# apache/paimon

Measured on NVIDIA H100. Metric: merged rows/sec at 16 runs x 40M rows, higher is better.
Workload: dtype int64

## Files before the change

paimon_b200/csrc/api.cu:

```cuda
#include <algorithm>
#include <atomic>
#include <cstdlib>
#include <cstring>
#include <map>
#include <memory>
#include <mutex>
#include <queue>

#include "pg_internal.h"

namespace pg {

static thread_local std::string g_last_error;
void set_error(const std::string &msg) { g_last_error = msg; }
pg_status fail(pg_status code, const std::string &msg) {
    g_last_error = msg;
    return code;
}

static int g_device = -1;

struct Arena {
    unsigned char *base = nullptr;
    size_t cap = 0;
// ... 334 lines not shown
    for (int c = 0; c < nc; c++) any |= read[c] && is_varlen(schema->field(c).type);
    if (!any) return PG_OK;
    for (int r = 0; r < (int)run_rows.size(); r++) {
        OutColumn *o = &out[(size_t)r * nc];
        const int64_t *bytes = &payload[(size_t)r * nc];
        auto carve = [&](void *base) {
            Carver cv(base);
            for (int c = 0; c < nc; c++)
                if (read[c] && is_varlen(schema->field(c).type)) o[c].data = cv.take<uint8_t>((size_t)bytes[c] + kReadPast);
            return cv.bytes();
        };
        const size_t total = carve(nullptr);
        Run &run = *scratch.runs[r];
        run.bufs.emplace_back(total);
        unsigned char *pl = run.bufs.back().get();
        if (!pl) return oom(who, "the var-len payload of a run", total);
        carve(pl);
        for (int c = 0; c < nc; c++) {
            if (!read[c] || !is_varlen(schema->field(c).type)) continue;
            run.varlen_bytes[c] = bytes[c];
            decoded_bytes += bytes[c];
        }
    }
    return PG_OK;
}

void RunBuilder::finish(uint64_t *out_runs, int64_t bytes_h2d, pg_section_info *info) {
    const int n_runs = (int)run_rows.size();
    for (int r = 0; r < n_runs; r++) {
        Run &run = *scratch.runs[r];
        for (int c = 0; c < nc; c++) {
            const OutColumn &o = out[(size_t)r * nc + c];
            if (read[c]) run.cols[c] = DevColumn{o.data ? o.data : run.bufs[0].get(), o.offsets, (const uint8_t *)o.validity};
        }
        run.bytes_h2d = r == 0 ? bytes_h2d : 0;
        out_runs[r] = g_runs.put(std::move(scratch.runs[r]));
    }
    if (info) {
        memset(info, 0, sizeof(*info));
        for (int64_t n : run_rows) info->n_rows += n;
        info->n_runs = n_runs;
        info->decoded_bytes = decoded_bytes;
    }
}

SectionFrame::SectionFrame(std::shared_ptr<const Schema> s, int n_runs, const char *who)
    : stream(copy_stream()), scratch(stream), b(std::move(s), n_runs, scratch, who) {}

pg_status SectionFrame::start(const uint8_t *read_cols, const char *const *names) {
    PG_CUDA(cudaEventCreate(&tm.e0));
    PG_CUDA(cudaEventCreate(&tm.e1));
    PG_CUDA(cudaEventRecord(tm.e0, stream));
    return b.read_columns(read_cols, names);
}

pg_status SectionFrame::place(const pg_file_desc *files, int n_files) {
    d_file.assign(n_files, nullptr);
    for (int f = 0; f < n_files; f++) {
        file_bytes += files[f].size;
        if (files[f].mem == PG_MEM_DEVICE) { d_file[f] = files[f].bytes; continue; }
        { pg_status st = file_image(scratch, files[f].bytes, files[f].size, b.who, &d_file[f]); if (st) return st; }
        h2d += files[f].size;
    }
    return PG_OK;
}

pg_status SectionFrame::finish(const int32_t *d_err, uint64_t *out_runs, pg_section_info *info) {
    PG_CUDA(cudaEventRecord(tm.e1, stream));
    int32_t herr = 0;
    SmallReads rb(stream);
    { pg_status rs = rb.add(&herr, d_err, 4); if (!rs) rs = rb.finish(); if (rs) return rs; }
    PG_CUDA(cudaGetLastError());
    { pg_status st = kernel_error(herr, b.who); if (st) return st; }
    b.finish(out_runs, h2d, info);
    if (info) {
        info->file_bytes = file_bytes;
        info->page_bytes = page_bytes;
        info->n_files = (int32_t)d_file.size();
        info->launches = launches;
        info->ms_decode = tm.ms();
    }
    return PG_OK;
}

static void free_outputs(Merge *m, bool release_memory = false) {
    m->out_cols.clear();
    m->has_batch = false;
    if (release_memory) {
        if (m->stream) cudaStreamSynchronize(m->stream);
        m->outbuf.release();
    }
}


static bool agg_supports_retract(int agg) {
    return agg == PG_AGG_SUM || agg == PG_AGG_PRODUCT || agg == PG_AGG_LAST_VALUE ||
           agg == PG_AGG_LAST_NON_NULL_VALUE || agg == PG_AGG_PRIMARY_KEY;
}

static pg_status build_descriptors(Merge *m) {
    const Schema *s = m->spec->schema.get();
    const Spec *sp = m->spec.get();
    if (s->n_key < 1 || s->n_key > PG_MAX_KEY_FIELDS)
        return fail(PG_ERR_UNSUPPORTED, "more than 4 primary-key fields are not implemented on the device");
    m->key = KeyDesc{};
    m->key.n_fields = s->n_key;
    int key_bytes = 0;
    bool all_fixed = true;
    for (int f = 0; f < s->n_key; f++) {
        int t = s->key_fields[f].type;
        if (t == PG_FLOAT || t == PG_DOUBLE)
            return fail(PG_ERR_UNSUPPORTED, "FLOAT / DOUBLE primary keys are not implemented on the device "
                                            "(the reference's comparator treats NaN as equal to everything)");
        m->key.type[f] = t;
        m->key.width[f] = type_width(t);
        if (is_varlen(t)) all_fixed = false;
        key_bytes += type_width(t);
    }
    m->key.exact = all_fixed && key_bytes <= 8;
    m->seq = SeqFields{};
    if (sp->seq_fields.size() > 4)
        return fail(PG_ERR_UNSUPPORTED, "more than 4 'sequence.field' columns are not implemented on the device");
    for (size_t i = 0; i < sp->seq_fields.size(); i++) {
        int vf = sp->seq_fields[i];
        if (vf < 0 || vf >= s->n_val) return fail(PG_ERR_INVALID, "sequence.field index out of range");
        int t = s->val_fields[vf].type;
        if (is_varlen(t))
            return fail(PG_ERR_UNSUPPORTED, "var-len 'sequence.field' columns are not implemented on the device");
        m->seq.col[i] = s->n_key + 2 + vf;
        m->seq.type[i] = t;
        m->seq.width[i] = type_width(t);
    }
    m->seq.n = (int32_t)sp->seq_fields.size();
    m->seq.ascending = sp->seq_ascending ? 1 : 0;
    m->flags = MergeFlags{sp->engine, sp->ignore_delete, sp->remove_record_on_delete, sp->drop_delete};

    const int nc = s->n_cols();
    m->cols.assign(nc, ColDesc{});
    m->varlen_cols.clear();
    m->emit.assign(nc, 1);
    for (int c = s->n_key + 2; c < nc; c++)
        if (!sp->read_fields.empty() && !sp->read_fields[c - s->n_key - 2]) m->emit[c] = 0;
    std::vector<uint8_t> needed = m->emit;
    for (int32_t vf : sp->seq_fields) if (vf >= 0 && vf < s->n_val) needed[s->n_key + 2 + vf] = 1;
    for (int32_t vf : sp->group_seq_fields) if (vf >= 0 && vf < s->n_val) needed[s->n_key + 2 + vf] = 1;
    for (int r = 0; r < m->k; r++)
        for (int c = 0; c < nc; c++)
            if (needed[c] && m->runs[r]->n_rows > 0 && !m->runs[r]->cols[c].data && !m->runs[r]->cols[c].offsets)
                return fail(PG_ERR_INVALID, "run " + std::to_string(r) + " has no buffers for column " + std::to_string(c) +
                                            ", which the merge reads (read-type projection dropped a field the merge "
                                            "function compares or emits)");
    for (int c = 0; c < nc; c++) {
        pg_field f = s->field(c);
        ColDesc &cd = m->cols[c];
        cd.type = f.type;
        cd.width = type_width(f.type);
        cd.nullable = f.nullable;
        cd.agg = PG_AGG_NONE;
        cd.retract = RT_OK;
        cd.varlen_index = -1;
        cd.decimal = 0;
        if (is_varlen(f.type) && m->emit[c]) {
            cd.varlen_index = (int)m->varlen_cols.size();
            m->varlen_cols.push_back(c);
        }
        if (c < s->n_key) { cd.mode = CM_KEY; cd.nullable = 0; }
        else if (c == s->n_key) { cd.mode = CM_SEQ; cd.nullable = 0; }
        else if (c == s->n_key + 1) { cd.mode = CM_KIND; cd.nullable = 0; }
        else {
            int vi = c - s->n_key - 2;
            int agg = sp->agg.empty() ? PG_AGG_NONE : sp->agg[vi];
            bool ign = !sp->ignore_retract.empty() && sp->ignore_retract[vi];
            const int32_t dec = sp->decimal.empty() ? 0 : sp->decimal[vi];
            const int32_t fold_dec = agg == PG_AGG_SUM || agg == PG_AGG_PRODUCT ? dec : 0;
            if (sp->engine == PG_ENGINE_AGGREGATE) {
                if (agg == PG_AGG_NONE) agg = PG_AGG_LAST_NON_NULL_VALUE;
                bool numeric = f.type == PG_INT8 || f.type == PG_INT16 || f.type == PG_INT32 ||
                               f.type == PG_INT64 || f.type == PG_FLOAT || f.type == PG_DOUBLE;
                if ((agg == PG_AGG_SUM || agg == PG_AGG_PRODUCT) && !numeric)
                    return fail(PG_ERR_INVALID, "sum/product need a numeric column");
                if ((agg == PG_AGG_BOOL_AND || agg == PG_AGG_BOOL_OR) && f.type != PG_BOOL)
                    return fail(PG_ERR_INVALID, "bool_and/bool_or need a BOOLEAN column");
                if ((agg == PG_AGG_MAX || agg == PG_AGG_MIN) && f.type == PG_BOOL)
                    return fail(PG_ERR_INVALID, "Incomparable type: BOOLEAN");
                if (agg < PG_AGG_SUM || agg > PG_AGG_PRIMARY_KEY)
                    return fail(PG_ERR_UNSUPPORTED, "aggregate function not implemented on the device");
                cd.mode = CM_FOLD;
                cd.agg = agg;
                cd.decimal = fold_dec;
                cd.nullable = 1;
                cd.retract = ign ? RT_IGNORE : (agg_supports_retract(agg) ? RT_OK : RT_ERROR);
            } else {
                const bool in_group = sp->n_groups() > 0 && sp->field_group[vi] >= 0;
                if (sp->engine == PG_ENGINE_PARTIAL_UPDATE && !in_group && agg != PG_AGG_NONE &&
                    agg != PG_AGG_LAST_NON_NULL_VALUE && agg != PG_AGG_PRIMARY_KEY)
                    return fail(PG_ERR_INVALID, "Must use sequence group for aggregation functions");
                cd.mode = CM_SELECT;
                if (sp->n_groups() > 0 && sp->field_group[vi] >= 0) {
                    const int g = sp->field_group[vi];
                    bool is_seq = false;
                    for (int j = sp->group_seq_start[g]; j < sp->group_seq_start[g + 1]; j++)
                        if (sp->group_seq_fields[j] == vi) is_seq = true;
                    cd.mode = is_seq ? CM_GSEQ : CM_GVAL;
                    cd.agg = g;
                    cd.nullable = 1;
                    if (!is_seq && agg != PG_AGG_NONE) {
                        cd.mode = CM_GAGG;
                        cd.agg = agg;
                        cd.decimal = fold_dec;
                        cd.group = g;
                        cd.retract = ign ? RT_IGNORE : (agg_supports_retract(agg) ? RT_OK : RT_ERROR);
                        m->has_group_aggs = true;
                    }
                }
            }
        }
    }

    const int k = m->k, nk = s->n_key, nv = (int)m->varlen_cols.size();
    MergeDesc h;
    const size_t total = h.carve(nullptr, k, nk, nc, nv);
    std::vector<unsigned char> host(total, 0);
    h.carve(host.data(), k, nk, nc, nv);
    m->varlen_bound.assign(nv, 0);
    for (int r = 0; r < k; r++) {
        const Run *run = m->runs[r].get();
        for (int f = 0; f < nk; f++) {
            h.key_ptrs[r * nk + f] = run->cols[f].data;
            h.key_offs[r * nk + f] = run->cols[f].offsets;
        }
        h.seq_ptrs[r] = (const int64_t *)run->cols[nk].data;
        h.kind_ptrs[r] = (const int8_t *)run->cols[nk + 1].data;
        for (int c = 0; c < nc; c++) {
            h.data[(size_t)c * k + r] = run->cols[c].data;
            h.offsets[(size_t)c * k + r] = run->cols[c].offsets;
            h.validity[(size_t)c * k + r] = (const uint32_t *)run->cols[c].validity;
            if (m->cols[c].varlen_index >= 0) m->varlen_bound[m->cols[c].varlen_index] += run->varlen_bytes[c];
        }
        h.run_rows[r] = run->n_rows;
    }
    memcpy(h.cols, m->cols.data(), sizeof(ColDesc) * nc);
    {
        int n = 0;
        for (int c = 0; c < nc; c++) if (m->emit[c] && m->cols[c].width == 0) h.col_order[n++] = c;
        for (int c = 0; c < nc; c++) if (m->emit[c] && m->cols[c].width != 0) h.col_order[n++] = c;
        m->n_passes = n;
        for (int v = 0; v < nv; v++) h.varlen_cols[v] = m->varlen_cols[v];
    }
    if (sp->n_groups() > 0) {
        SeqGroups *sg = h.groups;
        sg->n = sp->n_groups();
        for (int g = 0; g <= sg->n; g++) sg->start[g] = sp->group_seq_start[g];
        for (int j = 0; j < sp->group_seq_start[sg->n]; j++) {
            const int vf = sp->group_seq_fields[j];
            sg->col[j] = s->n_key + 2 + vf;
            sg->type[j] = s->val_fields[vf].type;
            sg->width[j] = type_width(s->val_fields[vf].type);
        }
        for (int g = 0; g < sg->n; g++) sg->partial_delete[g] = sp->group_partial_delete[g];
    }
    if (!m->d_desc || total > m->desc_cap) {
        if (m->d_desc) cudaFree(m->d_desc);
        m->d_desc = nullptr;
        PG_CUDA(cudaMalloc(&m->d_desc, total));
        m->desc_cap = total;
    }
    { pg_status ts = small_h2d(m->d_desc, host.data(), total, m->stream, m->ring); if (ts) return ts; }
    PG_CUDA(cudaStreamSynchronize(m->stream));
    m->desc.carve(m->d_desc, k, nk, nc, nv);
    if (sp->n_groups() == 0) m->desc.groups = nullptr;
    if (!m->h_totals) PG_CUDA(cudaMallocHost((void **)&m->h_totals, sizeof(int64_t) * (nv + 1) + 16));
    m->h_err = (int32_t *)(m->h_totals + nv + 1);
    return PG_OK;
}

pg_status kernel_error(int code, const char *who) {
    static const struct { int code; pg_status st; const char *msg; } kErrors[] = {
        {KERR_PU_DELETE, PG_ERR_MERGE_FUNCTION,
         "By default, Partial update can not accept delete records, you can choose one of the "
         "following solutions:\n1. Configure 'ignore-delete' to ignore delete records.\n"
         "2. Configure 'partial-update.remove-record-on-delete' to remove the whole row when "
         "receiving delete records.\n3. Configure 'sequence-group's to retract partial columns. "
         "Also configure 'partial-update.remove-record-on-sequence-group' to remove the whole "
         "row when receiving deleted records of `specified sequence group`."},
        {KERR_FIRST_ROW_RETRACT, PG_ERR_MERGE_FUNCTION,
         "By default, First row merge engine can not accept DELETE/UPDATE_BEFORE records.\n"
         "You can config 'ignore-delete' to ignore the DELETE/UPDATE_BEFORE records."},
        {KERR_AGG_RETRACT, PG_ERR_MERGE_FUNCTION,
         "Aggregate function does not support retraction, If you allow this function to ignore "
         "retraction messages, you can configure 'fields.${field_name}.ignore-retract'='true'."},
        {KERR_DIV_ZERO, PG_ERR_MERGE_FUNCTION, "ArithmeticException: / by zero"},
        {KERR_DEC_DIV_ZERO, PG_ERR_MERGE_FUNCTION, "ArithmeticException: Division by zero"},
        {KERR_DEC_DIV_UNDEFINED, PG_ERR_MERGE_FUNCTION, "ArithmeticException: Division undefined"},
        {KERR_DEC_NON_TERMINATING, PG_ERR_MERGE_FUNCTION,
         "ArithmeticException: Non-terminating decimal expansion; no exact representable decimal result."},
        {KERR_TILE_OVERFLOW, PG_ERR_INTERNAL,
         "a merge tile overflowed (does a run contain duplicate keys? SortMergeReader.java:37 requires unique keys per reader)"},
        {KERR_OFFSET_OVERFLOW, PG_ERR_INTERNAL, "a var-len column exceeds 2 GiB of payload"},
        {KERR_BAD_PAGE, PG_ERR_FORMAT, "a page or stream does not decode (malformed file or unsupported encoding)"},
        {KERR_PQ_HEADER, PG_ERR_FORMAT, "malformed or truncated page header"},
        {KERR_PQ_NO_DICT, PG_ERR_FORMAT, "dictionary-encoded page without dictionary"},
        {KERR_PQ_ROWS, PG_ERR_FORMAT, "page row counts do not add up"},
        {KERR_PQ_DICT_ID, PG_ERR_FORMAT, "dictionary id outside the dictionary"},
        {KERR_PQ_ENCODING, PG_ERR_UNSUPPORTED,
         "a page uses a value encoding the device decoder does not implement (PLAIN, dictionary, DELTA_BINARY_PACKED "
         "integers and RLE booleans are decoded)"},
        {KERR_PQ_LEVELS, PG_ERR_UNSUPPORTED, "repetition levels / BIT_PACKED definition levels are not decoded on device"},
    };
    if (code == KERR_NONE) return PG_OK;
    for (const auto &e : kErrors)
        if (e.code == code) return fail(e.st, e.st == PG_ERR_MERGE_FUNCTION ? std::string(e.msg) : std::string(who) + ": " + e.msg);
    return fail(PG_ERR_INTERNAL, std::string(who) + ": unknown kernel error " + std::to_string(code));
}


static pg_status execute(Merge *m) {
    pg_status st = ensure_device();
    if (st) return st;
    cudaStream_t sm = m->stream;
    PG_HOST_MARKS("merge execute");
    free_outputs(m);
    for (size_t r = m->runs.size(); r < m->bound.size(); r++)
        if (!m->runs.emplace_back(m->bound[r].lock())) {
            m->runs.clear();
            return fail(PG_ERR_INVALID, "a run of this merge has been freed since it was merged: rebind first");
        }
    const Schema *s = m->spec->schema.get();
    const int k = m->k, nc = s->n_cols(), nv = (int)m->varlen_cols.size();
    m->stats = pg_stats{};
    m->stats.rows_in = m->n_in;
    int launches = 0;

    const int S = kSampleStride;
    const int q = kPlanTile / S - 2 * k;
    if (q < 1) return fail(PG_ERR_UNSUPPORTED, "too many runs for one merge call");
    std::vector<LevelView> views;
    std::vector<int64_t> level_total;
    {
        int64_t stride = 1;
        while (true) {
            LevelView lv{};
            lv.stride = stride;
            int64_t tot = 0;
            for (int r = 0; r < k; r++) {
                lv.row0[r] = m->row0[r];
                lv.count[r] = (m->runs[r]->n_rows - m->row0[r]) / stride;
                tot += lv.count[r];
            }
            views.push_back(lv);
            level_total.push_back(tot);
            if (tot <= kPlanTile) break;
            stride *= S;
        }
    }
    const int top = (int)views.size() - 1;
    std::vector<int> n_tiles(top + 1);
    n_tiles[top] = 1;
    for (int l = top - 1; l >= 0; l--) n_tiles[l] = (int)((level_total[l + 1] + q - 1) / q);
    m->stats.n_levels = top;
    m->stats.n_tiles = n_tiles[0];

    PG_CUDA(cudaMemsetAsync(m->desc.err, 0, sizeof(int32_t), sm));
    PG_CUDA(cudaEventRecord(m->ev[0], sm));

    MergeLaunch ml{k, m->key, KeySrc{m->desc.key_ptrs, m->desc.key_offs}, sm, m->desc.err, nullptr};
    const int T = n_tiles[0];
    int64_t N = m->n_in;
    for (int r = 0; r < k; r++) N += m->row0[r];
    int *d_skip = nullptr;
    std::vector<int64_t *> bounds(top + 1);
    std::vector<uint64_t *> sk(top + 1), sref(top + 1);
    uint16_t *plan = nullptr;
    uint32_t *gplan = nullptr, *gagg = nullptr;
    int32_t *tile_rows = nullptr;
    int64_t *tmp_seq = nullptr, *row_base = nullptr;
    int8_t *tmp_kind = nullptr;
    uint64_t *vl_state = nullptr;
    const size_t vl_words = (size_t)T * std::max(nv, 1);
    auto carve_work = [&](void *base) {
        Carver cv(base);
        if (!m->key.exact) d_skip = cv.take<int>(1);
        for (int l = top; l >= 0; l--) {
            bounds[l] = cv.take<int64_t>((size_t)(n_tiles[l] + 1) * k);
            if (l > 0) {
                sk[l] = cv.take<uint64_t>((size_t)std::max<int64_t>(level_total[l], 1));
                sref[l] = cv.take<uint64_t>((size_t)std::max<int64_t>(level_total[l], 1));
            }
        }
        plan = cv.take<uint16_t>((size_t)N + 8);
        if (m->desc.groups) gplan = cv.take<uint32_t>((size_t)N + 4);
        if (m->has_group_aggs) gagg = cv.take<uint32_t>((size_t)N + 4);
        tile_rows = cv.take<int32_t>(T);
        tmp_seq = cv.take<int64_t>((size_t)N + 2);
        tmp_kind = cv.take<int8_t>((size_t)N + 16);
        row_base = cv.take<int64_t>(T);
        vl_state = cv.take<uint64_t>(vl_words);
        return cv.bytes();
    };
    PG_CUDA(m->work.reserve(carve_work(nullptr)));
    carve_work(m->work.base);

    if (!m->key.exact) {
        launch_key_lcp(ml, views[0], d_skip);
        ml.skip = d_skip;
        launches++;
    }
    for (int l = top; l >= 0; l--) {
        launch_partition(ml, views[l], l < top ? sk[l + 1] : nullptr, l < top ? sref[l + 1] : nullptr, q, n_tiles[l],
                         bounds[l]);
        launches++;
        if (l > 0) {
            launch_merge_keys(ml, views[l], bounds[l], n_tiles[l], sk[l], sref[l]);
            launches++;
        }
    }
    PG_CUDA(cudaEventRecord(m->ev[1], sm));

    PG_CUDA(cudaMemsetAsync(vl_state, 0, sizeof(uint64_t) * vl_words, sm));
    PG_CUDA(cudaMemsetAsync(m->desc.tile_counter, 0, sizeof(int32_t), sm));

    PlanArgs pa{};
    pa.bounds = bounds[0];
    pa.n_tiles = T;
    pa.seq_ptrs = m->desc.seq_ptrs;
    pa.kind_ptrs = m->desc.kind_ptrs;
    pa.flags = m->flags;
    pa.seq = m->seq;
    pa.ptrs = m->desc.ptrs();
    pa.plan = plan;
    pa.tile_rows = tile_rows;
    pa.tmp_seq = tmp_seq;
    pa.tmp_kind = tmp_kind;
    pa.groups = m->desc.groups;
    pa.gplan = gplan;
    pa.gagg = gagg;
    launch_plan(ml, pa);
    launch_scan(sm, tile_rows, T, row_base, m->desc.totals);
    launches += 2;
    PG_CUDA(cudaEventRecord(m->ev[2], sm));
    PG_HOST_MARK("enqueue");
    {
        SmallReads rb(sm);
        pg_status rs = rb.add(m->h_totals, m->desc.totals, sizeof(int64_t));
        if (!rs) rs = rb.add(m->h_err, m->desc.err, sizeof(int32_t));
        if (!rs) rs = rb.finish();
        if (rs) return rs;
    }
    if (*m->h_err != KERR_NONE) return kernel_error(*m->h_err, "merge");
    PG_HOST_MARK("size_readback");

    const int64_t n_out = m->h_totals[0];
    m->n_out = n_out;
    m->out_cols.assign(nc, pg_out_column{});
    size_t vspan = 0;
    int64_t bytes_out = 0;
    auto carve_out = [&](void *base) {
        Carver cv(base);
        bytes_out = 0;
        for (int c = 0; c < nc; c++)
            if (m->cols[c].nullable && m->emit[c]) {
                m->out_cols[c].validity = cv.take<uint8_t>((size_t)((n_out + 31) / 32) * 4 + kReadPast);
                bytes_out += (n_out + 7) / 8;
            }
        vspan = cv.bytes();
        for (int c = 0; c < nc; c++) {
            const ColDesc &cd = m->cols[c];
            pg_out_column &oc = m->out_cols[c];
            if (!m->emit[c]) continue;
            if (cd.width > 0) {
                oc.data_bytes = n_out * cd.width;
                oc.data = cv.take<uint8_t>((size_t)oc.data_bytes + kReadPast);
                bytes_out += oc.data_bytes;
            } else {
                oc.data_bytes = m->varlen_bound[cd.varlen_index];
                oc.data = cv.take<uint8_t>((size_t)oc.data_bytes + kReadPast);
                oc.offsets = cv.take<int32_t>((size_t)n_out + 1 + kReadPast / 4);
                bytes_out += 4 * (n_out + 1);
            }
        }
        return cv.bytes();
    };
    PG_CUDA(m->outbuf.reserve(carve_out(nullptr)));
    carve_out(m->outbuf.base);
    if (vspan) PG_CUDA(cudaMemsetAsync(m->outbuf.base, 0, vspan, sm));
    m->stats.bytes_out = bytes_out;
    { pg_status ts = small_h2d(m->desc.out_cols, m->out_cols.data(), sizeof(pg_out_column) * nc, sm, m->ring); if (ts) return ts; }

    EmitArgs ea{};
    ea.bounds = bounds[0];
    ea.n_tiles = (T + 1) / 2;
    ea.n_plan_tiles = T;
    ea.tile_rows = tile_rows;
    ea.k = k;
    ea.plan = plan;
    ea.row_base = row_base;
    ea.tmp_seq = tmp_seq;
    ea.tmp_kind = tmp_kind;
    ea.gplan = gplan;
    ea.gagg = gagg;
    ea.cols = m->desc.cols;
    ea.col_order = m->desc.col_order;
    ea.n_passes = m->n_passes;
    ea.varlen_cols = m->desc.varlen_cols;
    ea.ptrs = m->desc.ptrs();
    ea.run_rows = m->desc.run_rows;
    ea.n_cols = nc;
    ea.n_varlen = nv;
    ea.out_cols = m->desc.out_cols;
    ea.totals = m->desc.totals;
    ea.vl_state = vl_state;
    ea.tile_counter = m->desc.tile_counter;
    ea.err = m->desc.err;
    ea.stream = sm;
    PG_CUDA(cudaEventRecord(m->ev[4], sm));
    launch_emit(ea);
    launches++;
    PG_CUDA(cudaEventRecord(m->ev[3], sm));
    PG_HOST_MARK("alloc_emit");
    {
        SmallReads rb(sm);
        pg_status rs = rb.add(m->h_err, m->desc.err, sizeof(int32_t));
        if (!rs) rs = rb.add(m->h_totals, m->desc.totals, sizeof(int64_t) * (nv + 1));
        if (!rs) rs = rb.finish();
        if (rs) return rs;
    }
    PG_CUDA(cudaGetLastError());
    PG_HOST_MARK("emit_readback");
    m->has_batch = true;
    if (*m->h_err != KERR_NONE) {
        free_outputs(m);
        return kernel_error(*m->h_err, "merge");
    }
    for (int c = 0; c < nc; c++)
        if (m->cols[c].width == 0 && m->emit[c]) {
            m->out_cols[c].data_bytes = m->h_totals[1 + m->cols[c].varlen_index];
            m->stats.bytes_out += m->out_cols[c].data_bytes;
        }
    m->stats.rows_out = n_out;
    m->stats.launches = launches;
    cudaEventElapsedTime(&m->stats.ms_partition, m->ev[0], m->ev[1]);
    cudaEventElapsedTime(&m->stats.ms_plan, m->ev[1], m->ev[2]);
    cudaEventElapsedTime(&m->stats.ms_alloc, m->ev[2], m->ev[4]);
    cudaEventElapsedTime(&m->stats.ms_emit, m->ev[4], m->ev[3]);
    cudaEventElapsedTime(&m->stats.ms_total, m->ev[0], m->ev[3]);
    m->runs.clear();
    return PG_OK;
}

}


using namespace pg;

extern "C" {

const char *pg_last_error(void) { return g_last_error.c_str(); }
int32_t pg_abi_version(void) { return PG_ABI_VERSION; }

pg_status pg_init(int32_t device_ordinal) {
    int n = 0;
    cudaError_t e = cudaGetDeviceCount(&n);
    if (e != cudaSuccess || n == 0)
        return fail(PG_ERR_CUDA, std::string("no CUDA device: libpaimon_gpu has no CPU fallback (") +
                                     cudaGetErrorString(e) + ")");
    if (device_ordinal < 0 || device_ordinal >= n) return fail(PG_ERR_INVALID, "bad device ordinal");
    if (g_device >= 0 && g_device != device_ordinal)
        return fail(PG_ERR_INVALID, "pg_init: this process is already bound to device " + std::to_string(g_device) +
                                    " (one process per GPU: handles, streams and cached buffers belong to it)");
    PG_CUDA(cudaSetDevice(device_ordinal));
    g_device = device_ordinal;
    cudaMemPool_t pool;
    PG_CUDA(cudaDeviceGetDefaultMemPool(&pool, device_ordinal));
    uint64_t thr = UINT64_MAX;
    PG_CUDA(cudaMemPoolSetAttribute(pool, cudaMemPoolAttrReleaseThreshold, &thr));
    return PG_OK;
}

pg_status pg_shutdown(void) {
    if (g_device >= 0) {
        cudaSetDevice(g_device);
        cudaDeviceSynchronize();
        buf_trim(0);
        cudaMemPool_t pool;
        if (cudaDeviceGetDefaultMemPool(&pool, g_device) == cudaSuccess) cudaMemPoolTrimTo(pool, 0);
    }
    return PG_OK;
}

pg_status pg_schema_create(const pg_schema_desc *desc, uint64_t *out_schema) {
    if (!desc || !out_schema) return fail(PG_ERR_INVALID, "null argument");
    if (desc->n_key < 1 || desc->n_val < 0 || desc->n_key + 2 + desc->n_val > kMaxCols)
        return fail(PG_ERR_INVALID, "bad field counts");
    auto s = std::make_unique<Schema>();
    s->n_key = desc->n_key;
    s->n_val = desc->n_val;
    for (int i = 0; i < desc->n_key; i++) {
        if (!type_ok(desc->key_fields[i].type)) return fail(PG_ERR_INVALID, "bad key field type");
        s->key_fields.push_back(pg_field{desc->key_fields[i].type, 0});
    }
    for (int i = 0; i < desc->n_val; i++) {
        if (!type_ok(desc->val_fields[i].type)) return fail(PG_ERR_INVALID, "bad value field type");
        s->val_fields.push_back(desc->val_fields[i]);
    }
    *out_schema = g_schemas.put(std::move(s));
    return PG_OK;
}
// ... 493 lines not shown
```

paimon_b200/csrc/parquet_decode.cu:

```cuda
#include <algorithm>
#include <cstring>
#include <memory>
#include <stdexcept>

#include "device_utils.cuh"
#include "parquet_meta.h"
#include "inflate_device.cuh"
#include "lz4_device.cuh"
#include "snappy_device.cuh"
#include "scan_kernels.cuh"
#include "zstd_device.cuh"

namespace pg {

enum : int { ENC_PLAIN = 0, ENC_DICT = 1, ENC_DELTA_BP = 2, ENC_RLE_BOOL = 3 };

struct PqChunk {
    const uint8_t *base;
    int64_t avail;
    int64_t num_values;
    int64_t row0;
    int32_t col, run, file, codec;
    int32_t max_def, phys, phys_width;
    int32_t cast;
    int32_t n_pages, n_dicts;
    int64_t scratch_bytes;
    int64_t dict_entries;
    int64_t ids_entries;
    int64_t page_bytes;
    int32_t page_base, dict_base;
    int64_t scratch_base, dict_entry_base, ids_base;
};

struct PqPage {
    const uint8_t *src;
    const uint8_t *body;
    uint8_t *aux;
    int32_t src_len, body_len;
    int32_t num_values, chunk;
    int8_t type, enc, compressed, bad;
    int32_t def_len;
    int64_t row0;
    int32_t values_off, nnz;
    int64_t ids_base;
    int64_t payload_bytes;
    int64_t payload_base;
    int64_t vs_base;
    int32_t is_last, pad;
    int64_t entry_base;
};

struct PqOut {
    void *data;
    int32_t *offsets;
    uint32_t *validity;
    int32_t out_width;
    int32_t is_bool;
};

struct PqPair {
    int32_t run, col, chunk0, chunk1;
    int64_t vs_rows_base;
    int32_t idx, pad;
};

__device__ __forceinline__ uint32_t pq_varint(const uint8_t *&p, const uint8_t *end, bool &ok) {
    uint32_t v = 0;
    int shift = 0;
    while (p < end) {
        uint8_t b = *p++;
        v |= (uint32_t)(b & 0x7f) << shift;
        if (!(b & 0x80)) return v;
        shift += 7;
    }
    ok = false;
    return v;
}


struct TRd {
    const uint8_t *p, *end;
    int bad;
    __host__ __device__ uint32_t byte() {
        if (p >= end) { bad = 1; return 0; }
        return *p++;
    }
    __host__ __device__ uint64_t varint() {
        uint64_t v = 0;
        for (int sh = 0; sh < 70; sh += 7) {
            const uint32_t b = byte();
            v |= (uint64_t)(b & 0x7f) << sh;
            if (!(b & 0x80)) return v;
        }
        bad = 1;
        return v;
    }
    __host__ __device__ int64_t zz() {
        const uint64_t v = varint();
        return (int64_t)(v >> 1) ^ -(int64_t)(v & 1);
    }
    __host__ __device__ int field(int &id) {
        const uint32_t h = byte();
        if (h == 0 || bad) return 0;
        const int d = (int)(h >> 4);
        if (d == 0) id = (int)zz(); else id += d;
        return (int)(h & 15);
    }
    __host__ __device__ void advance(uint64_t n) {
        if ((uint64_t)(end - p) < n) { bad = 1; p = end; } else p += n;
    }
    __host__ __device__ void skip_flat(int t, bool in_container) {
        switch (t) {
            case 1: case 2: if (in_container) byte(); return;
            case 3: byte(); return;
            case 4: case 5: case 6: varint(); return;
            case 7: advance(8); return;
            case 8: advance(varint()); return;
            case 9: case 10: {
                const uint32_t h = byte();
                const int et = (int)(h & 15);
                uint64_t n = h >> 4;
                if (n == 15) n = varint();
                if (et == 9 || et == 10 || et == 11 || et == 12) { if (n) bad = 1; return; }
                for (uint64_t i = 0; i < n && !bad; i++) skip_flat(et, true);
                return;
            }
            case 11: { if (varint() != 0) bad = 1; return; }
            default: bad = 1; return;
        }
    }
    __host__ __device__ void skip(int t) {
        if (t != 12) { skip_flat(t, false); return; }
        int depth = 1;
        while (depth > 0 && !bad) {
            const uint32_t h = byte();
            if (h == 0) { depth--; continue; }
            if ((h >> 4) == 0) zz();
            const int ft = (int)(h & 15);
            if (ft == 12) depth++; else skip_flat(ft, false);
        }
    }
};

struct PqHeader {
    int type, unc, comp, nv, enc, def_enc, def_len, rep_len, is_compressed, hdr;
};

__host__ __device__ inline bool pq_parse_header(const uint8_t *p, const uint8_t *end, PqHeader &h) {
    TRd r{p, end, 0};
    h.type = -1; h.unc = 0; h.comp = 0; h.nv = 0; h.enc = 0; h.def_enc = pq::E_RLE; h.def_len = 0; h.rep_len = 0;
    h.is_compressed = 1;
    int id = 0, t;
    while ((t = r.field(id)) != 0 && !r.bad) {
        if (id == 1 && t == 5) h.type = (int)r.zz();
        else if (id == 2 && t == 5) h.unc = (int)r.zz();
        else if (id == 3 && t == 5) h.comp = (int)r.zz();
        else if ((id == 5 || id == 7 || id == 8) && t == 12) {
            const int outer = id;
            int i2 = 0, t2;
            while ((t2 = r.field(i2)) != 0 && !r.bad) {
                if (outer == 8) {
                    if (i2 == 1 && t2 == 5) h.nv = (int)r.zz();
                    else if (i2 == 4 && t2 == 5) h.enc = (int)r.zz();
                    else if (i2 == 5 && t2 == 5) h.def_len = (int)r.zz();
                    else if (i2 == 6 && t2 == 5) h.rep_len = (int)r.zz();
                    else if (i2 == 7 && (t2 == 1 || t2 == 2)) h.is_compressed = t2 == 1;
                    else r.skip(t2);
                } else {
                    if (i2 == 1 && t2 == 5) h.nv = (int)r.zz();
                    else if (i2 == 2 && t2 == 5) h.enc = (int)r.zz();
                    else if (i2 == 3 && t2 == 5 && outer == 5) h.def_enc = (int)r.zz();
                    else r.skip(t2);
                }
            }
        } else r.skip(t);
    }
    h.hdr = (int)(r.p - p);
    return !r.bad && h.type >= 0;
}

__device__ __forceinline__ void pq_err(int32_t *err, int code) { atomicCAS(err, KERR_NONE, code); }
__host__ __device__ __forceinline__ int64_t pq_al64(int64_t x) { return (x + 63) & ~(int64_t)63; }
__host__ __device__ __forceinline__ int64_t pq_min64(int64_t a, int64_t b) { return a < b ? a : b; }

template <bool FILL>
__host__ __device__ inline int pq_walk_chunk(PqChunk *chunks, int c, PqPage *pages, PqPage *dicts, uint8_t *scratch) {
    const PqChunk ch = chunks[c];
    const uint8_t *p = ch.base, *end = ch.base + ch.avail;
    int64_t vals = 0, sc = 0, dict_entries = 0, page_bytes = 0;
    int n_pages = 0, n_dicts = 0;
    int code = KERR_NONE;
    bool needs_ids = false;
    const bool codec_on = ch.codec != pq::C_UNCOMPRESSED;
    while (vals < ch.num_values) {
        PqHeader h;
        if (p >= end || !pq_parse_header(p, end, h)) { code = KERR_PQ_HEADER; break; }
        const uint8_t *body = p + h.hdr;
        if (h.comp < 0 || h.unc < 0 || h.nv < 0 || (int64_t)(end - body) < (int64_t)h.comp) { code = KERR_PQ_HEADER; break; }
        if (h.type == pq::P_DICTIONARY) {
            if (n_dicts > 0 || n_pages > 0 || (h.enc != pq::E_PLAIN && h.enc != pq::E_PLAIN_DICTIONARY)) {
                code = KERR_PQ_ENCODING;
                break;
            }
            const int body_len = codec_on ? h.unc : h.comp;
            if ((int64_t)h.nv * ch.phys_width > (int64_t)body_len) { code = KERR_BAD_PAGE; break; }
            if (FILL) {
                PqPage d;
                memset(&d, 0, sizeof(d));
                d.src = body; d.src_len = h.comp; d.body_len = body_len;
                d.body = codec_on ? scratch + ch.scratch_base + sc : body;
                d.num_values = h.nv; d.chunk = c; d.type = (int8_t)pq::P_DICTIONARY; d.compressed = codec_on;
                d.entry_base = ch.dict_entry_base;
                dicts[ch.dict_base] = d;
            }
            if (codec_on) sc += pq_al64((int64_t)h.unc + 16);
            if (ch.phys == pq::T_BYTE_ARRAY) dict_entries += h.nv;
            page_bytes += body_len;
            n_dicts++;
        } else if (h.type == pq::P_DATA || h.type == pq::P_DATA_V2) {
            int enc = -1;
            if (h.enc == pq::E_PLAIN) enc = ENC_PLAIN;
            else if (h.enc == pq::E_PLAIN_DICTIONARY || h.enc == pq::E_RLE_DICTIONARY) enc = ENC_DICT;
            else if (h.enc == pq::E_DELTA_BINARY_PACKED && (ch.phys == pq::T_INT32 || ch.phys == pq::T_INT64)) enc = ENC_DELTA_BP;
            else if (h.enc == pq::E_RLE && ch.phys == pq::T_BOOLEAN) enc = ENC_RLE_BOOL;
            if (enc < 0 || (enc == ENC_DICT && ch.phys == pq::T_BOOLEAN)) { code = KERR_PQ_ENCODING; break; }
            if (enc == ENC_DICT && n_dicts == 0) { code = KERR_PQ_NO_DICT; break; }
            const bool v2 = h.type == pq::P_DATA_V2;
            if ((v2 && h.rep_len != 0) || (!v2 && ch.max_def > 0 && h.def_enc != pq::E_RLE) || (v2 && h.def_len < 0)) {
                code = KERR_PQ_LEVELS;
                break;
            }
            const bool compressed = codec_on && (!v2 || h.is_compressed);
            const int body_len = compressed ? h.unc : h.comp;
            const int64_t unc_need = compressed ? pq_al64((int64_t)h.unc + 16) : 0;
            const int64_t aux_need = enc == ENC_DELTA_BP ? pq_al64((int64_t)body_len + (int64_t)h.nv * ch.phys_width + 16) : 0;
            if (FILL) {
                PqPage g;
                memset(&g, 0, sizeof(g));
                g.src = body; g.src_len = h.comp; g.body_len = body_len;
                g.body = compressed ? scratch + ch.scratch_base + sc : body;
                g.aux = aux_need ? scratch + ch.scratch_base + sc + unc_need : nullptr;
                g.num_values = h.nv; g.chunk = c; g.type = (int8_t)h.type; g.enc = (int8_t)enc; g.compressed = compressed;
                g.def_len = v2 ? h.def_len : 0;
                g.row0 = ch.row0 + vals;
                g.ids_base = ch.ids_base + vals;
                pages[ch.page_base + n_pages] = g;
            }
            sc += unc_need + aux_need;
            if (enc == ENC_DICT || enc == ENC_RLE_BOOL) needs_ids = true;
            page_bytes += body_len;
            vals += h.nv;
            n_pages++;
        }
        p = body + h.comp;
    }
    if (code == KERR_NONE && vals != ch.num_values) code = KERR_PQ_ROWS;
    if (!FILL) {
        PqChunk &o = chunks[c];
        o.n_pages = n_pages; o.n_dicts = n_dicts; o.scratch_bytes = sc; o.dict_entries = dict_entries;
        o.ids_entries = needs_ids ? ch.num_values : 0;
        o.page_bytes = page_bytes;
    }
    return code;
}

template <bool FILL>
__global__ void k_pq_walk(PqChunk *chunks, int n_chunks, PqPage *pages, PqPage *dicts, uint8_t *scratch, int32_t *err) {
    const int c = blockIdx.x * blockDim.x + threadIdx.x;
    if (c >= n_chunks) return;
    const int code = pq_walk_chunk<FILL>(chunks, c, pages, dicts, scratch);
    if (code != KERR_NONE) pq_err(err, code);
}

constexpr int kScanThreads = 512;
__global__ void __launch_bounds__(kScanThreads) k_pq_chunk_scan(PqChunk *chunks, int n, int64_t *totals) {
    __shared__ int64_t part[6][kScanThreads];
    const int per = (n + kScanThreads - 1) / kScanThreads;
    const int b = threadIdx.x * per, e = min(b + per, n);
    int64_t s[6] = {0, 0, 0, 0, 0, 0};
    for (int i = b; i < e; i++) {
        s[0] += chunks[i].n_pages; s[1] += chunks[i].n_dicts; s[2] += chunks[i].scratch_bytes;
        s[3] += chunks[i].dict_entries; s[4] += chunks[i].ids_entries; s[5] += chunks[i].page_bytes;
    }
    for (int q = 0; q < 6; q++) part[q][threadIdx.x] = s[q];
    __syncthreads();
    if (threadIdx.x < 6) {
        int64_t acc = 0;
        for (int i = 0; i < kScanThreads; i++) { const int64_t t = part[threadIdx.x][i]; part[threadIdx.x][i] = acc; acc += t; }
        totals[threadIdx.x] = acc;
    }
    __syncthreads();
    for (int q = 0; q < 6; q++) s[q] = part[q][threadIdx.x];
    for (int i = b; i < e; i++) {
        PqChunk &c = chunks[i];
        c.page_base = (int32_t)s[0]; c.dict_base = (int32_t)s[1]; c.scratch_base = s[2]; c.dict_entry_base = s[3];
        c.ids_base = s[4];
        s[0] += c.n_pages; s[1] += c.n_dicts; s[2] += c.scratch_bytes; s[3] += c.dict_entries; s[4] += c.ids_entries;
    }
}

__global__ void k_pq_snappy_lz4(const PqPage *pages, int n_pages, const PqPage *dicts, int n_dicts, const PqChunk *chunks,
                                int32_t *err) {
    const int w = (int)(((int64_t)blockIdx.x * blockDim.x + threadIdx.x) >> 5), lane = threadIdx.x & 31;
    if (w >= n_pages + n_dicts) return;
    const PqPage &pg = w < n_pages ? pages[w] : dicts[w - n_pages];
    const int codec = chunks[pg.chunk].codec;
    if (!pg.compressed || (codec != pq::C_SNAPPY && codec != pq::C_LZ4)) return;
    const int prefix = pg.type == pq::P_DATA_V2 ? pg.def_len : 0;
    uint8_t *out0 = const_cast<uint8_t *>(pg.body);
    const uint8_t *in0 = pg.src;
    if (prefix > pg.src_len || prefix > pg.body_len) { if (lane == 0) pq_err(err, KERR_BAD_PAGE); return; }
    for (int i = lane; i < prefix; i += 32) out0[i] = in0[i];
    const uint8_t *src = in0 + prefix;
    uint8_t *dst = out0 + prefix;
    const int n_src = pg.src_len - prefix, n_dst = pg.body_len - prefix;
    if (codec == pq::C_LZ4) {
        if (lz4::decode_hadoop(src, n_src, dst, n_dst) != n_dst && lane == 0) pq_err(err, KERR_BAD_PAGE);
        return;
    }
    if (snappy::decode(src, n_src, dst, n_dst) != n_dst && lane == 0) pq_err(err, KERR_BAD_PAGE);
}

constexpr int kZsWarps = 4;
__global__ void __launch_bounds__(kZsWarps * 32)
k_pq_zstd(const PqPage *pages, int n_pages, const PqPage *dicts, int n_dicts, const PqChunk *chunks, uint8_t *lit_scratch,
          int32_t *counter, int32_t *err) {
    __shared__ zs::Tables T[kZsWarps];
    static_assert(sizeof(inflate::Tables) <= sizeof(zs::Tables), "tables overlay");
    const int w = threadIdx.x >> 5, lane = threadIdx.x & 31;
    uint8_t *lit = lit_scratch + ((size_t)blockIdx.x * kZsWarps + w) * (size_t)(zs::kMaxBlock + 64);
    while (true) {
        int j = 0;
        if (lane == 0) j = atomicAdd(counter, 1);
        j = __shfl_sync(0xffffffffu, j, 0);
        if (j >= n_pages + n_dicts) return;
        const PqPage &pg = j < n_pages ? pages[j] : dicts[j - n_pages];
        const int codec = chunks[pg.chunk].codec;
        if (!pg.compressed || (codec != pq::C_ZSTD && codec != pq::C_GZIP)) continue;
        const int prefix = pg.type == pq::P_DATA_V2 ? pg.def_len : 0;
        uint8_t *out0 = const_cast<uint8_t *>(pg.body);
        if (prefix > pg.src_len || prefix > pg.body_len) { if (lane == 0) pq_err(err, KERR_BAD_PAGE); continue; }
        for (int i = lane; i < prefix; i += 32) out0[i] = pg.src[i];
        const int64_t want = pg.body_len - prefix;
        const int64_t got = codec == pq::C_ZSTD
            ? zs::decode(pg.src + prefix, pg.src_len - prefix, out0 + prefix, want, lit, T[w])
            : inflate::inflate_gzip(pg.src + prefix, pg.src_len - prefix, out0 + prefix, want, *(inflate::Tables *)&T[w]);
        if (got != want && lane == 0) pq_err(err, KERR_BAD_PAGE);
        __syncwarp();
    }
}

__device__ __forceinline__ uint64_t dl_varint(const uint8_t *p, int n, int &pos) {
    uint64_t v = 0;
    for (int sh = 0; pos < n && sh < 70; sh += 7) {
        const uint8_t b = p[pos++];
        v |= (uint64_t)(b & 0x7f) << sh;
        if (!(b & 0x80)) break;
    }
    return v;
}
__global__ void k_pq_delta(PqPage *pages, int n_pages, const PqChunk *chunks, int32_t *err) {
    const int w = (int)(((int64_t)blockIdx.x * blockDim.x + threadIdx.x) >> 5), lane = threadIdx.x & 31;
    if (w >= n_pages) return;
    const PqPage pg = pages[w];
    if (pg.enc != ENC_DELTA_BP) return;
    const PqChunk &ch = chunks[pg.chunk];
    const int width = ch.phys_width;
    int prefix = 0;
    if (ch.max_def > 0) {
        if (pg.type == pq::P_DATA_V2) prefix = pg.def_len;
        else if (pg.body_len >= 4)
            prefix = 4 + (int)((uint32_t)pg.body[0] | ((uint32_t)pg.body[1] << 8) | ((uint32_t)pg.body[2] << 16) | ((uint32_t)pg.body[3] << 24));
        else prefix = -1;
    }
    if (prefix < 0 || prefix > pg.body_len) { if (lane == 0) { pq_err(err, KERR_BAD_PAGE); pages[w].bad = 1; } return; }
    for (int i = lane; i < prefix; i += 32) pg.aux[i] = pg.body[i];
    const uint8_t *p = pg.body + prefix;
    const int n = pg.body_len - prefix;
    uint8_t *out = pg.aux + prefix;
    int pos = 0;
    const int block_size = (int)dl_varint(p, n, pos);
    const int n_mini = (int)dl_varint(p, n, pos);
    const int64_t total = (int64_t)dl_varint(p, n, pos);
    const uint64_t zz = dl_varint(p, n, pos);
    uint64_t last = (zz >> 1) ^ (0 - (zz & 1));
    bool bad = n_mini <= 0 || block_size <= 0 || block_size % n_mini != 0 || total > pg.num_values || total < 0;
    const int mini = bad ? 1 : block_size / n_mini;
    if (!bad && total > 0 && lane == 0) {
        if (width == 8) memcpy(out, &last, 8); else { uint32_t x = (uint32_t)last; memcpy(out, &x, 4); }
    }
    int64_t done = 1;
    while (!bad && done < total) {
        const uint64_t mz = dl_varint(p, n, pos);
        const uint64_t min_delta = (mz >> 1) ^ (0 - (mz & 1));
        const int bw_pos = pos;
        pos += n_mini;
        if (pos > n) { bad = true; break; }
        for (int m = 0; m < n_mini && done < total; m++) {
            const int bw = p[bw_pos + m];
            if (bw > 64 || pos + (int64_t)mini * bw / 8 > n) { bad = true; break; }
            for (int v0 = 0; v0 < mini && done < total; v0 += 32) {
                const int v = v0 + lane;
                uint64_t d = 0;
                if (v < mini && bw > 0) {
                    const int64_t bit = (int64_t)v * bw;
                    const uint8_t *q = p + pos + (bit >> 3);
                    const int sh = (int)(bit & 7);
                    uint64_t lo = 0;
                    const int nb = (sh + bw + 7) >> 3;
                    for (int b = 0; b < nb && b < 8; b++) lo |= (uint64_t)q[b] << (8 * b);
                    d = lo >> sh;
                    if (nb > 8) d |= (uint64_t)q[8] << (64 - sh);
                    if (bw < 64) d &= ((uint64_t)1 << bw) - 1;
                }
                uint64_t x = v < mini ? d + min_delta : 0;
#pragma unroll
                for (int o = 1; o < 32; o <<= 1) {
                    const uint64_t y = __shfl_up_sync(0xffffffffu, x, o);
                    if (lane >= o) x += y;
                }
                const uint64_t val = last + x;
                const int64_t idx = done + lane;
                if (v < mini && idx < total) {
                    if (width == 8) memcpy(out + idx * 8, &val, 8);
                    else { uint32_t t = (uint32_t)val; memcpy(out + idx * 4, &t, 4); }
                }
                const int cnt = min(32, mini - v0);
                last = __shfl_sync(0xffffffffu, val, cnt - 1);
                done += cnt;
            }
            pos += mini * bw / 8;
        }
    }
    if (lane == 0) {
        if (bad) { pq_err(err, KERR_BAD_PAGE); pages[w].bad = 1; }
        pages[w].body = pg.aux;
        pages[w].body_len = prefix + (int)(total > 0 && !bad ? total : 0) * width;
    }
}

__device__ int pq_def_to_bits(const uint8_t *p, const uint8_t *end, int count, uint32_t *bm, int64_t row0, bool &ok) {
    const int lane = threadIdx.x & 31;
    int pos = 0, nnz = 0;
    while (pos < count) {
        if (p >= end) { ok = false; break; }
// ... 408 lines not shown
        const int sh = (int)(a & 7) * 8;
        const uint64_t lo = q[0];
        return sh ? (lo >> sh) | (q[1] << (64 - sh)) : lo;
    }
    const uintptr_t a = (uintptr_t)p;
    const uint32_t *q = (const uint32_t *)(a & ~(uintptr_t)3);
    const int sh = (int)(a & 3) * 8;
    const uint32_t lo = q[0];
    return sh ? (uint64_t)((lo >> sh) | (q[1] << (32 - sh))) : (uint64_t)lo;
}

template <bool kPlainStrings> struct PqPlainStage {
    int vs[2][kExpThreads + 4];
    int bnd[kPayBatches + 1];
    alignas(16) uint8_t in[2][kPayIn];
    alignas(16) uint8_t out[kPayOut];
};
template <> struct PqPlainStage<false> {};

template <bool kPlainStrings>
__global__ void __launch_bounds__(kExpThreads, 6)
k_pq_expand(const PqPage *pages, const PqPage *dicts, const PqChunk *chunks, const PqOut *outs, int n_cols,
            const int32_t *ids, const int32_t *vstart, const int32_t *dict_off, const int32_t *dict_len) {
    __shared__ uint32_t s_bits[kExpThreads];
    __shared__ int s_rank[kExpThreads];
    __shared__ int s_wlen[kExpThreads];
    __shared__ int s_ws[34];
    __shared__ PqPlainStage<kPlainStrings> stage;
    const PqPage pg = pages[blockIdx.x];
    if (pg.bad || pg.num_values == 0) return;
    const PqChunk ch = chunks[pg.chunk];
    if (kPlainStrings != (ch.phys == pq::T_BYTE_ARRAY && pg.enc == ENC_PLAIN)) return;
    const PqOut out = outs[ch.run * n_cols + ch.col];
    const int tid = threadIdx.x, lane = tid & 31, warp = tid >> 5;
    const int64_t row0 = pg.row0, row1 = pg.row0 + pg.num_values;
    const int64_t g0 = row0 & ~(int64_t)31;
    const int n_words = (int)((row1 - g0 + 31) >> 5);
    const uint8_t *values = pg.body + pg.values_off;
    const int pw = ch.phys_width;
    const bool varlen = ch.phys == pq::T_BYTE_ARRAY;
    const bool is_dict = pg.enc == ENC_DICT;
    const PqPage *dj = is_dict ? &dicts[ch.dict_base] : nullptr;
    const uint8_t *dbody = is_dict ? dj->body : nullptr;
    const int64_t ebase = is_dict ? dj->entry_base : 0;
    const int32_t *pids = ids + pg.ids_base;
    const int32_t *vs = vstart + pg.vs_base;
    uint8_t *payload = varlen ? (uint8_t *)out.data : nullptr;
    int carry_rank = 0;
    int64_t carry_bytes = pg.payload_base;
    for (int w0 = 0; w0 < n_words; w0 += kExpThreads) {
        const int jw = w0 + tid;
        uint32_t bits = 0;
        if (jw < n_words) {
            const int64_t wrow = g0 + 32 * (int64_t)jw;
            const int lo = wrow < row0 ? (int)(row0 - wrow) : 0;
            const int64_t hi = pq_min64(32, row1 - wrow);
            const uint32_t mask = (hi >= 32 ? 0xffffffffu : ((1u << hi) - 1)) & ~((1u << lo) - 1);
            bits = out.validity ? (out.validity[wrow >> 5] & mask) : mask;
        }
        int tot = 0;
        const int excl = block_scan_excl(__popc(bits), s_ws, &tot);
        s_bits[tid] = bits;
        s_rank[tid] = carry_rank + excl;
        __syncthreads();
        const int nw = min(kExpThreads, n_words - w0);
        if (varlen && is_dict) {
            for (int jj = warp; jj < nw; jj += kExpThreads / 32) {
                const uint32_t b = s_bits[jj];
                int len = 0;
                if ((b >> lane) & 1) len = dict_len[ebase + pids[s_rank[jj] + __popc(b & ((1u << lane) - 1))]];
#pragma unroll
                for (int d = 16; d > 0; d >>= 1) len += __shfl_xor_sync(0xffffffffu, len, d);
                if (lane == 0) s_wlen[jj] = len;
            }
            __syncthreads();
            int wtot = 0;
            const int wl = tid < nw ? s_wlen[tid] : 0;
            const int wex = block_scan_excl(wl, s_ws, &wtot);
            s_wlen[tid] = wex;
            __syncthreads();
            for (int jj = warp; jj < nw; jj += kExpThreads / 32) {
                const uint32_t b = s_bits[jj];
                const int64_t row = g0 + 32 * (int64_t)(w0 + jj) + lane;
                const bool inpage = row >= row0 && row < row1;
                int len = 0;
                const uint8_t *src = nullptr;
                if ((b >> lane) & 1) {
                    const int id = pids[s_rank[jj] + __popc(b & ((1u << lane) - 1))];
                    len = dict_len[ebase + id];
                    src = dbody + dict_off[ebase + id];
                }
                const int incl = warp_scan_incl(len);
                const int64_t off = carry_bytes + s_wlen[jj] + incl - len;
                if (inpage) out.offsets[row] = (int32_t)off;
                for (int r8 = 0; r8 < 32; r8 += 4) {
                    const int sl = r8 + (lane >> 3);
                    const int64_t o2 = __shfl_sync(0xffffffffu, off, sl);
                    const int l2 = __shfl_sync(0xffffffffu, len, sl);
                    const uint8_t *s2 = (const uint8_t *)__shfl_sync(0xffffffffu, (unsigned long long)(uintptr_t)src, sl);
                    for (int bb = lane & 7; bb < l2; bb += 8) payload[o2 + bb] = s2[bb];
                }
            }
            carry_bytes += wtot;
        } else {
            constexpr int kExpUnroll = 4, kStep = kExpThreads / 32;
            const int fmode = varlen ? 0 : pg.enc == ENC_RLE_BOOL ? 1 : ch.phys == pq::T_BOOLEAN ? 2 : is_dict ? 3 : 4;
            if (fmode == 4 && pw == 8 && out.out_width == 8 && ch.cast == 0) {
                constexpr int kPairUnroll = 2;
                const int half = lane >> 4, p0 = 2 * (lane & 15);
                const uintptr_t a0 = (uintptr_t)values;
                const int sh = (int)(a0 & 7) * 8;
                const uint64_t *q0 = (const uint64_t *)(a0 & ~(uintptr_t)7);
                uint64_t *od = (uint64_t *)out.data;
                for (int j0 = 2 * warp; j0 < nw; j0 += 2 * kStep * kPairUnroll) {
                    int64_t row[kPairUnroll];
                    bool in0[kPairUnroll], in1[kPairUnroll];
                    uint64_t l0[kPairUnroll], h0[kPairUnroll], l1[kPairUnroll], h1[kPairUnroll];
#pragma unroll
                    for (int u = 0; u < kPairUnroll; u++) {
                        const int jj = j0 + 2 * kStep * u + half;
                        const uint32_t b = jj < nw ? s_bits[jj] : 0;
                        const int rk = jj < nw ? s_rank[jj] + __popc(b & ((1u << p0) - 1)) : 0;
                        const bool v0 = (b >> p0) & 1, v1 = (b >> (p0 + 1)) & 1;
                        row[u] = g0 + 32 * (int64_t)(w0 + jj) + p0;
                        in0[u] = jj < nw && row[u] >= row0 && row[u] < row1;
                        in1[u] = jj < nw && row[u] + 1 >= row0 && row[u] + 1 < row1;
                        const int r1 = rk + (v0 ? 1 : 0);
                        l0[u] = v0 ? q0[rk] : 0;
                        h0[u] = (v0 && sh) ? q0[rk + 1] : 0;
                        l1[u] = v1 ? q0[r1] : 0;
                        h1[u] = (v1 && sh) ? q0[r1 + 1] : 0;
                    }
#pragma unroll
                    for (int u = 0; u < kPairUnroll; u++) {
                        const uint64_t x0 = sh ? (l0[u] >> sh) | (h0[u] << (64 - sh)) : l0[u];
                        const uint64_t x1 = sh ? (l1[u] >> sh) | (h1[u] << (64 - sh)) : l1[u];
                        if (in0[u] && in1[u]) *(ulonglong2 *)(od + row[u]) = make_ulonglong2(x0, x1);
                        else if (in0[u]) od[row[u]] = x0;
                        else if (in1[u]) od[row[u] + 1] = x1;
                    }
                }
            } else
            for (int j0 = warp; j0 < nw; j0 += kStep * kExpUnroll) {
                int64_t row[kExpUnroll];
                int rank[kExpUnroll];
                bool inpage[kExpUnroll], valid[kExpUnroll];
#pragma unroll
                for (int u = 0; u < kExpUnroll; u++) {
                    const int jj = j0 + u * kStep;
                    const uint32_t b = jj < nw ? s_bits[jj] : 0;
                    row[u] = g0 + 32 * (int64_t)(w0 + jj) + lane;
                    inpage[u] = jj < nw && row[u] >= row0 && row[u] < row1;
                    valid[u] = (b >> lane) & 1;
                    rank[u] = jj < nw ? s_rank[jj] + __popc(b & ((1u << lane) - 1)) : 0;
                }
                if (fmode == 0) {
                    int32_t o[kExpUnroll];
#pragma unroll
                    for (int u = 0; u < kExpUnroll; u++) o[u] = inpage[u] ? vs[rank[u]] : 0;
#pragma unroll
                    for (int u = 0; u < kExpUnroll; u++) if (inpage[u]) out.offsets[row[u]] = o[u];
                    continue;
                }
                uint64_t v[kExpUnroll];
                if (fmode == 4) {
                    if (pw == 8) {
                        const uintptr_t a0 = (uintptr_t)values;
                        const int sh = (int)(a0 & 7) * 8;
                        const uint64_t *q0 = (const uint64_t *)(a0 & ~(uintptr_t)7);
                        uint64_t lo[kExpUnroll], hi[kExpUnroll];
#pragma unroll
                        for (int u = 0; u < kExpUnroll; u++) {
                            const bool ld = inpage[u] && valid[u];
                            lo[u] = ld ? q0[rank[u]] : 0;
                            hi[u] = (ld && sh) ? q0[rank[u] + 1] : 0;
                        }
#pragma unroll
                        for (int u = 0; u < kExpUnroll; u++) v[u] = sh ? (lo[u] >> sh) | (hi[u] << (64 - sh)) : lo[u];
                    } else {
                        const uintptr_t a0 = (uintptr_t)values;
                        const int sh = (int)(a0 & 3) * 8;
                        const uint32_t *q0 = (const uint32_t *)(a0 & ~(uintptr_t)3);
                        uint32_t lo[kExpUnroll], hi[kExpUnroll];
#pragma unroll
                        for (int u = 0; u < kExpUnroll; u++) {
                            const bool ld = inpage[u] && valid[u];
                            lo[u] = ld ? q0[rank[u]] : 0;
                            hi[u] = (ld && sh) ? q0[rank[u] + 1] : 0;
                        }
#pragma unroll
                        for (int u = 0; u < kExpUnroll; u++) v[u] = __funnelshift_r(lo[u], hi[u], sh);
                    }
                } else if (fmode == 3) {
                    int32_t id[kExpUnroll];
#pragma unroll
                    for (int u = 0; u < kExpUnroll; u++) id[u] = (inpage[u] && valid[u]) ? pids[rank[u]] : -1;
#pragma unroll
                    for (int u = 0; u < kExpUnroll; u++) v[u] = id[u] >= 0 ? pq_load_unaligned(dbody + (int64_t)id[u] * pw, pw) : 0;
                } else {
#pragma unroll
                    for (int u = 0; u < kExpUnroll; u++) {
                        v[u] = 0;
                        if (inpage[u] && valid[u])
                            v[u] = fmode == 1 ? (uint64_t)(pids[rank[u]] & 1) : (uint64_t)((values[rank[u] >> 3] >> (rank[u] & 7)) & 1);
                    }
                }
#pragma unroll
                for (int u = 0; u < kExpUnroll; u++) {
                    if (!inpage[u]) continue;
                    uint64_t x = valid[u] ? v[u] : 0;
                    if (valid[u] && ch.cast == 1) x = (uint64_t)(int64_t)(int32_t)(uint32_t)x;
                    else if (valid[u] && ch.cast == 2) x = (uint64_t)__double_as_longlong((double)__uint_as_float((uint32_t)x));
                    store_fixed(out.data, out.out_width, row[u], x);
                }
            }
        }
        carry_rank += tot;
        __syncthreads();
    }
    if (varlen) {
        if constexpr (kPlainStrings) {
            auto &s_vs = stage.vs;
            auto &s_bnd = stage.bnd;
            auto &s_in = stage.in;
            auto &s_out = stage.out;
            const int nnz = pg.nnz;
            const int64_t pb = pg.payload_base;
            const int nb = (nnz + kExpThreads - 1) / kExpThreads;
            const bool staged_page = nb <= kPayBatches;
            __syncthreads();
            if (staged_page) for (int i = tid; i <= nb; i += kExpThreads) s_bnd[i] = vs[min(i * kExpThreads, nnz)];
            __syncthreads();
            auto batch_src = [&](int b2) -> const uint8_t * { return values + ((int64_t)s_bnd[b2] - pb) + 4 * (int64_t)b2 * kExpThreads; };
            auto batch_fits = [&](int b2) -> bool {
                const int jn = min(kExpThreads, nnz - b2 * kExpThreads);
                const int out_len = s_bnd[b2 + 1] - s_bnd[b2];
                const int iskew = (int)((uintptr_t)batch_src(b2) & 15), oskew = (int)((uintptr_t)(payload + s_bnd[b2]) & 15);
                return iskew + out_len + 4 * jn <= kPayIn && oskew + out_len <= kPayOut;
            };
            auto prefetch = [&](int b2) {
                const int jn = min(kExpThreads, nnz - b2 * kExpThreads);
                int *dv = s_vs[b2 & 1];
                for (int i = tid; i <= jn; i += kExpThreads) cp_async4(dv + i, vs + b2 * kExpThreads + i);
                if (batch_fits(b2)) {
                    const uint8_t *src0 = batch_src(b2);
                    const int iskew = (int)((uintptr_t)src0 & 15);
                    const int n16 = (iskew + (s_bnd[b2 + 1] - s_bnd[b2]) + 4 * jn + 15) >> 4;
                    uint8_t *di = s_in[b2 & 1];
                    for (int i = tid; i < n16; i += kExpThreads) cp_async16(di + 16 * i, src0 - iskew + 16 * i);
                }
                cp_async_commit();
            };
            if (staged_page && nb > 0) prefetch(0);
            for (int b2 = 0; b2 < nb; b2++) {
                const int j0 = b2 * kExpThreads, jn = min(kExpThreads, nnz - j0);
                if (!staged_page) {
                    for (int t = tid >> 3; t < jn; t += kExpThreads / 8) {
                        const int st = vs[j0 + t], len = vs[j0 + t + 1] - st;
                        const uint8_t *src = values + ((int64_t)st - pb) + 4 * (int64_t)(j0 + t + 1);
                        for (int b3 = tid & 7; b3 < len; b3 += 8) payload[(int64_t)st + b3] = src[b3];
                    }
                    continue;
                }
                if (b2 + 1 < nb) { prefetch(b2 + 1); cp_async_wait<1>(); } else cp_async_wait<0>();
                __syncthreads();
                const int *cvs = s_vs[b2 & 1];
                const int out0 = s_bnd[b2], out_len = s_bnd[b2 + 1] - out0;
                if (batch_fits(b2)) {
                    const uint8_t *src0 = batch_src(b2);
                    const int iskew = (int)((uintptr_t)src0 & 15), oskew = (int)((uintptr_t)(payload + out0) & 15);
                    if (tid < jn) {
                        const int o = cvs[tid] - out0, len = cvs[tid + 1] - cvs[tid];
                        const uint8_t *sp = s_in[b2 & 1] + iskew + o + 4 * (tid + 1);
                        uint8_t *dp = s_out + oskew + o;
                        for (int b3 = 0; b3 < len; b3++) dp[b3] = sp[b3];
                    }
                    __syncthreads();
                    uint8_t *dst16 = payload + out0 - oskew;
                    const int end = oskew + out_len;
                    for (int c = tid; c * 16 < end; c += kExpThreads) {
                        const int c0 = c * 16;
                        if (c0 >= oskew && c0 + 16 <= end) *(uint4 *)(dst16 + c0) = *(const uint4 *)(s_out + c0);
                        else for (int b3 = max(c0, oskew); b3 < min(c0 + 16, end); b3++) dst16[b3] = s_out[b3];
                    }
                } else {
                    for (int t = tid >> 3; t < jn; t += kExpThreads / 8) {
                        const int st = cvs[t], len = cvs[t + 1] - st;
                        const uint8_t *src = values + ((int64_t)st - pb) + 4 * (int64_t)(j0 + t + 1);
                        for (int b3 = tid & 7; b3 < len; b3 += 8) payload[(int64_t)st + b3] = src[b3];
                    }
                }
                __syncthreads();
            }
        }
        if (pg.is_last && tid == 0) out.offsets[row1] = (int32_t)(pg.payload_base + pg.payload_bytes);
    }
}

__global__ void k_pq_zero_first_offset(const PqOut *outs, int n) {
    const int i = blockIdx.x * blockDim.x + threadIdx.x;
    if (i < n && outs[i].offsets) outs[i].offsets[0] = 0;
}


static int phys_cast(int pg_t, int phys) {
    switch (pg_t) {
        case PG_INT8: case PG_INT16: case PG_INT32: return phys == pq::T_INT32 ? 0 : -1;
        case PG_INT64: return phys == pq::T_INT64 ? 0 : (phys == pq::T_INT32 ? 1 : -1);
        case PG_FLOAT: return phys == pq::T_FLOAT ? 0 : -1;
        case PG_DOUBLE: return phys == pq::T_DOUBLE ? 0 : (phys == pq::T_FLOAT ? 2 : -1);
        case PG_BOOL: return phys == pq::T_BOOLEAN ? 0 : -1;
        case PG_STRING: case PG_BINARY: return phys == pq::T_BYTE_ARRAY ? 0 : -1;
        default: return -1;
    }
}
static int phys_width_of(int phys) {
    return phys == pq::T_INT32 || phys == pq::T_FLOAT ? 4 : (phys == pq::T_INT64 || phys == pq::T_DOUBLE ? 8 : 0);
}

static pg_status map_file_schema(RunBuilder &b, const pq::FileMetaData &m, int run) {
    if (m.schema.empty()) return fail(PG_ERR_FORMAT, "parquet: empty schema");
    const int nleaf = (int)m.schema.size() - 1;
    if (m.schema[0].num_children != nleaf)
        return fail(PG_ERR_UNSUPPORTED, "parquet: nested columns are not decoded on device (flat KeyValue file schemas are)");
    std::vector<std::string> cols(nleaf);
    for (int i = 1; i <= nleaf; i++) {
        if (m.schema[i].num_children != 0 || m.schema[i].repetition == pq::R_REPEATED)
            return fail(PG_ERR_UNSUPPORTED, "parquet: nested / repeated column " + m.schema[i].name);
        cols[i - 1] = m.schema[i].name;
    }
    { pg_status st = b.add_file(run, m.num_rows, cols); if (st) return st; }
    for (int c = 0; c < b.nc; c++) {
        const int fc = b.file_col.back()[c];
        if (fc < 0) continue;
        const pq::SchemaElement &e = m.schema[fc + 1];
        if (phys_cast(b.schema->field(c).type, e.type) < 0)
            return fail(PG_ERR_UNSUPPORTED, "parquet: column " + e.name + " has a physical type the device decoder "
                                            "does not map to the table type");
    }
    for (const pq::RowGroup &g : m.row_groups) {
        if ((int)g.columns.size() != nleaf) return fail(PG_ERR_FORMAT, "parquet: row group with a different column count");
        for (const pq::ColumnChunk &cc : g.columns)
            if (cc.codec != pq::C_UNCOMPRESSED && cc.codec != pq::C_SNAPPY && cc.codec != pq::C_ZSTD && cc.codec != pq::C_GZIP &&
                cc.codec != pq::C_LZ4)
                return fail(PG_ERR_UNSUPPORTED, "parquet: compression codec " + std::to_string(cc.codec) +
                                                " is not decoded on device (UNCOMPRESSED, SNAPPY, ZSTD, GZIP and Hadoop-framed LZ4 = 5 are); write with "
                                                "'file.compression'='zstd' / 'snappy' / 'gzip' / 'lz4' / 'none' or let the Java side decompress");
    }
    return PG_OK;
}

struct ChunkTables {
    std::vector<PqChunk> chunks;
    std::vector<PqPair> pairs;
    bool any_snappy = false, any_lz4 = false, any_delta = false, any_zstd = false;
    int64_t pair_rows = 0;
};

static pg_status build_chunk_tables(const Schema *s, const pg_file_desc *files, const std::vector<const uint8_t *> &d_file,
                                    const std::vector<const pq::FileMetaData *> &meta, const RunBuilder &b, ChunkTables &t) {
    const int nc = s->n_cols();
    const int n_runs = (int)b.run_rows.size();
    std::vector<std::vector<int>> run_files(n_runs);
    for (int f = 0; f < (int)meta.size(); f++) run_files[files[f].run].push_back(f);
    for (int r = 0; r < n_runs; r++) {
        for (int c = 0; c < nc; c++) {
            if (!b.read[c]) continue;
            const int chunk0 = (int)t.chunks.size();
            for (int f : run_files[r]) {
                const pq::FileMetaData &m = *meta[f];
                const int fc = b.file_col[f][c];
                int64_t rg_row0 = 0;
                int64_t rows = 0;
                if (fc < 0) continue;
                for (const pq::RowGroup &g : m.row_groups) {
                    const pq::ColumnChunk &cc = g.columns[fc];
                    const int64_t start = cc.start();
                    if (cc.num_values != g.num_rows) return fail(PG_ERR_FORMAT, "parquet: page row counts do not add up");
                    if (cc.num_values == 0) continue;
                    if (start < 4 || start >= files[f].size) return fail(PG_ERR_FORMAT, "parquet: page offset out of range");
                    PqChunk ch;
                    memset(&ch, 0, sizeof(ch));
                    ch.base = d_file[f] + start;
                    ch.avail = std::min<int64_t>(cc.total_compressed_size > 0 ? cc.total_compressed_size : files[f].size,
                                                 files[f].size - start);
                    ch.num_values = cc.num_values;
                    ch.row0 = b.file_row0[f] + rg_row0;
                    ch.col = c; ch.run = r; ch.file = f; ch.codec = cc.codec;
                    ch.max_def = m.schema[fc + 1].repetition == pq::R_OPTIONAL ? 1 : 0;
                    ch.phys = cc.type;
                    ch.phys_width = phys_width_of(cc.type);
                    ch.cast = phys_cast(s->field(c).type, cc.type);
                    if (cc.type != m.schema[fc + 1].type) return fail(PG_ERR_FORMAT, "parquet: column chunk type differs from the schema");
                    if (cc.codec == pq::C_SNAPPY) t.any_snappy = true;
                    if (cc.codec == pq::C_LZ4) t.any_lz4 = true;
                    if (cc.codec == pq::C_ZSTD || cc.codec == pq::C_GZIP) t.any_zstd = true;
                    for (int32_t e : cc.encodings) if (e == pq::E_DELTA_BINARY_PACKED) t.any_delta = true;
                    if (cc.num_values > 0) t.chunks.push_back(ch);
                    rg_row0 += g.num_rows;
                    rows += g.num_rows;
                }
                if (rows != m.num_rows) return fail(PG_ERR_FORMAT, "parquet: row group row counts do not add up");
            }
            if (is_varlen(s->field(c).type)) {
                PqPair pr{r, c, chunk0, (int)t.chunks.size(), t.pair_rows, (int)t.pairs.size(), 0};
                t.pairs.push_back(pr);
                t.pair_rows += b.run_rows[r];
            }
        }
    }
    return PG_OK;
}

#ifdef PG_WALK_TIMING
static void walk_timing_dump() {
    static long long h[kWtSlots][8];
    cudaDeviceSynchronize();
    cudaMemcpyFromSymbol(h, g_walk_ts, sizeof(h));
    double acc[3] = {0, 0, 0}, steps = 0, vals = 0, steps_max = 0;
    long long g_lo = LLONG_MAX, g_hi = 0;
    int n = 0;
    for (int s = 0; s < kWtSlots; s++) {
        if (h[s][4] == 0) continue;
        n++;
        for (int k = 0; k < 3; k++) acc[k] += (double)h[s][k];
        steps += (double)h[s][3];
        steps_max = std::max(steps_max, (double)h[s][3]);
        vals += (double)h[s][4];
        g_lo = std::min(g_lo, h[s][5]);
        g_hi = std::max(g_hi, h[s][6]);
    }
    if (n == 0) return;
    const double tot = acc[0] + acc[1] + acc[2];
    fprintf(stderr, "[walk timing] %d warps: cycles per step issue %.0f wait %.0f walk %.0f (%.1f / %.1f / %.1f %%); "
                    "steps per warp %.1f (max %.0f), values per lane-step %.2f, span %.3f ms\n",
            n, acc[0] / steps, acc[1] / steps, acc[2] / steps, 100 * acc[0] / tot, 100 * acc[1] / tot, 100 * acc[2] / tot,
            steps / n, steps_max, vals / (32.0 * steps), (g_hi - g_lo) * 1e-6);
    int hist[10] = {0};
    double busy = 0;
    for (int s = 0; s < kWtSlots; s++) {
        if (h[s][4] == 0) continue;
        hist[std::min(9, (int)(10.0 * (h[s][5] - g_lo) / (double)(g_hi - g_lo + 1)))]++;
        busy += (double)(h[s][6] - h[s][5]);
    }
    fprintf(stderr, "[walk timing] warp start by tenth of the span:");
    for (int i = 0; i < 10; i++) fprintf(stderr, " %d", hist[i]);
    fprintf(stderr, "; mean warp lifetime %.3f ms\n", busy / n * 1e-6);
    static long long z[kWtSlots][8];
    cudaMemcpyToSymbol(g_walk_ts, z, sizeof(z));
}
#endif

struct SideStream {
    cudaStream_t s = nullptr;
    cudaEvent_t fork = nullptr, tables = nullptr, join = nullptr;
};
static pg_status side_stream(SideStream **out) {
    static thread_local SideStream side;
    if (!side.s) {
        int prio_lo = 0, prio_hi = 0;
        cudaDeviceGetStreamPriorityRange(&prio_lo, &prio_hi);
        PG_CUDA(cudaStreamCreateWithPriority(&side.s, cudaStreamNonBlocking, prio_hi));
        PG_CUDA(cudaEventCreateWithFlags(&side.fork, cudaEventDisableTiming));
        PG_CUDA(cudaEventCreateWithFlags(&side.tables, cudaEventDisableTiming));
        PG_CUDA(cudaEventCreateWithFlags(&side.join, cudaEventDisableTiming));
    }
    *out = &side;
    return PG_OK;
}

struct SideSync {
    cudaStream_t s = nullptr;
    ~SideSync() { if (s) cudaStreamSynchronize(s); }
};

static pg_status decode_section(const std::shared_ptr<const Schema> &s, const pg_file_desc *files, int nf, int n_runs,
                                const char *const *names, const uint8_t *read_cols, uint64_t *out_runs,
                                pg_section_info *info, const pq::FileMetaData *footer0 = nullptr) {
    const int nc = s->n_cols();
    SectionFrame fr(s, n_runs, "parquet");
    SideSync side_sync;
    PG_HOST_MARKS("parquet decode_section");
    RunBuilder &b = fr.b;
    cudaStream_t sm = fr.stream;
    { pg_status st = fr.start(read_cols, names); if (st) return st; }

    { pg_status st = fr.place(files, nf); if (st) return st; }
    std::vector<pq::FileMetaData> own_meta(nf);
    std::vector<const pq::FileMetaData *> meta(nf, nullptr);
    if (footer0) meta[0] = footer0;
    DeviceRanges rd(sm, files, nf);
    try {
        if (!rd.files.empty()) {
            std::vector<pq::FileMetaData> m = pq::read_footers(rd, rd.sizes);
            for (size_t i = 0; i < rd.files.size(); i++) own_meta[rd.files[i]] = std::move(m[i]);
        }
        for (int f = 0; f < nf; f++) {
            if (meta[f]) continue;
            if (files[f].mem == PG_MEM_HOST) own_meta[f] = pq::parse_footer(files[f].bytes, files[f].size);
            meta[f] = &own_meta[f];
        }
    } catch (const std::exception &e) {
        return rd.st ? rd.st : fail(PG_ERR_FORMAT, e.what());
    }
    PG_HOST_MARK("footers");
    std::vector<uint8_t> any_optional(nc, 0);
    for (int f = 0; f < nf; f++) {
        pg_status st = map_file_schema(b, *meta[f], files[f].run);
        if (st) return st;
        for (int c = 0; c < nc; c++) {
            const int fc = b.file_col[f][c];
            if (fc == -1 || (fc >= 0 && meta[f]->schema[fc + 1].repetition == pq::R_OPTIONAL)) any_optional[c] = 1;
        }
    }
    { pg_status st = b.check_runs(); if (st) return st; }
    ChunkTables ct;
    { pg_status st = build_chunk_tables(s.get(), files, fr.d_file, meta, b, ct); if (st) return st; }
    const int n_chunks = (int)ct.chunks.size(), n_pairs = (int)ct.pairs.size();
    PG_HOST_MARK("chunk_tables");

    { pg_status st = b.alloc(any_optional, b.missing); if (st) return st; }
    std::vector<PqOut> outs((size_t)n_runs * nc);
    auto fill_outs = [&] {
        for (size_t i = 0; i < outs.size(); i++) {
            const int t = s->field((int)(i % nc)).type;
            outs[i] = PqOut{b.out[i].data, b.out[i].offsets, b.out[i].validity, type_width(t), t == PG_BOOL};
        }
    };
    fill_outs();
    const bool any_empty = std::find(b.run_rows.begin(), b.run_rows.end(), 0) != b.run_rows.end();

    PqChunk *d_chunks;
    PqOut *d_outs, *d_outs2;
    PqPair *d_pairs;
    int64_t *d_totals;
    auto carve_tables = [&](void *base) {
        Carver cv(base);
        d_chunks = cv.take<PqChunk>((size_t)std::max(n_chunks, 1));
        d_outs = cv.take<PqOut>(outs.size());
        d_outs2 = cv.take<PqOut>(outs.size());
        d_pairs = cv.take<PqPair>((size_t)std::max(n_pairs, 1));
        d_totals = cv.take<int64_t>(8 + (size_t)n_pairs);
        return cv.bytes();
    };
    const size_t tb_bytes = carve_tables(nullptr);
    void *tb = fr.scratch.take(tb_bytes);
    if (!tb) return oom("parquet", "the chunk tables", tb_bytes);
    carve_tables(tb);
    int32_t *d_err = (int32_t *)(d_totals + 6);
    PG_CUDA(cudaMemsetAsync(d_totals, 0, sizeof(int64_t) * (8 + (size_t)n_pairs), sm));
    if (n_chunks) { pg_status ts = small_h2d(d_chunks, ct.chunks.data(), sizeof(PqChunk) * n_chunks, sm); if (ts) return ts; }
    { pg_status ts = small_h2d(d_outs, outs.data(), sizeof(PqOut) * outs.size(), sm); if (ts) return ts; }
    if (n_pairs) { pg_status ts = small_h2d(d_pairs, ct.pairs.data(), sizeof(PqPair) * n_pairs, sm); if (ts) return ts; }
    int64_t h_tot[8] = {0, 0, 0, 0, 0, 0, 0, 0};
    PG_HOST_MARK("tables");
    if (n_chunks) {
        k_pq_walk<false><<<(n_chunks + 63) / 64, 64, 0, sm>>>(d_chunks, n_chunks, nullptr, nullptr, nullptr, d_err);
        k_pq_chunk_scan<<<1, kScanThreads, 0, sm>>>(d_chunks, n_chunks, d_totals);
        fr.launches += 2;
        {
            SmallReads rb(sm);
            pg_status rs = rb.add(h_tot, d_totals, sizeof(int64_t) * 8);
            if (!rs) rs = rb.finish();
            if (!rs) rs = kernel_error((int)(h_tot[6] & 0xffffffff), "parquet");
            if (rs) return rs;
        }
    }
    const int64_t n_pages = h_tot[0], n_dicts = h_tot[1], sc_bytes = h_tot[2], dict_entries = h_tot[3],
                  ids_entries = h_tot[4];
    fr.page_bytes = h_tot[5];
    PG_HOST_MARK("readback1");
    if (n_pages > 0x7fffffffLL) return fail(PG_ERR_UNSUPPORTED, "parquet: too many pages in one section");

    int zs_ctas = 0;
    if (ct.any_zstd) {
        int dev = 0, sms = 132;
        cudaGetDevice(&dev);
        cudaDeviceGetAttribute(&sms, cudaDevAttrMultiProcessorCount, dev);
        zs_ctas = (int)std::min<int64_t>((int64_t)sms * 5, (n_pages + n_dicts + kZsWarps - 1) / kZsWarps);
    }
    PqPage *d_pages, *d_dicts;
    uint8_t *d_sc, *d_zs_lit;
    int32_t *d_dict_off, *d_dict_len, *d_ids, *d_vstart;
    auto carve_pages = [&](void *base) {
        Carver cv(base);
        d_pages = cv.take<PqPage>((size_t)std::max<int64_t>(n_pages, 1));
        d_dicts = cv.take<PqPage>((size_t)std::max<int64_t>(n_dicts, 1));
        d_sc = cv.take<uint8_t>((size_t)sc_bytes + kReadPast);
        d_dict_off = cv.take<int32_t>((size_t)dict_entries + 1);
        d_dict_len = cv.take<int32_t>((size_t)dict_entries + 1);
        d_ids = cv.take<int32_t>((size_t)ids_entries + 1);
        d_vstart = cv.take<int32_t>((size_t)(ct.pair_rows + n_pages + n_pairs + 2));
        d_zs_lit = cv.take<uint8_t>((size_t)zs_ctas * kZsWarps * (size_t)(zs::kMaxBlock + 64));
        return cv.bytes();
    };
    const size_t sb_bytes = carve_pages(nullptr);
    void *sbuf = fr.scratch.take(sb_bytes);
    if (!sbuf) return oom("parquet", "the page table and scratch", sb_bytes);
    carve_pages(sbuf);
    const int np = (int)n_pages, nd = (int)n_dicts;
    std::vector<int64_t> pair_tot(std::max(n_pairs, 1), 0);
    if (np > 0) {
        k_pq_walk<true><<<(n_chunks + 63) / 64, 64, 0, sm>>>(d_chunks, n_chunks, d_pages, d_dicts, d_sc, d_err);
        fr.launches++;
        if (ct.any_snappy || ct.any_lz4) {
            const int64_t th = (int64_t)(np + nd) * 32;
            k_pq_snappy_lz4<<<(unsigned)((th + 127) / 128), 128, 0, sm>>>(d_pages, np, d_dicts, nd, d_chunks, d_err);
            fr.launches++;
        }
        if (ct.any_zstd && zs_ctas > 0) {
            k_pq_zstd<<<zs_ctas, kZsWarps * 32, 0, sm>>>(d_pages, np, d_dicts, nd, d_chunks, d_zs_lit, (int32_t *)(d_totals + 7), d_err);
            fr.launches++;
        }
        if (ct.any_delta) {
            k_pq_delta<<<(unsigned)(((int64_t)np * 32 + 127) / 128), 128, 0, sm>>>(d_pages, np, d_chunks, d_err);
            fr.launches++;
        }
        if (dict_entries > 0) {
            k_pq_walk_dicts<<<(nd + kWalkWarps - 1) / kWalkWarps, kWalkWarps * 32, 0, sm>>>(
                d_dicts, nd, d_chunks, d_dict_off, d_dict_len, d_err);
            fr.launches++;
        }
        k_pq_levels<<<(unsigned)(((int64_t)np * 32 + 127) / 128), 128, 0, sm>>>(d_pages, np, d_dicts, d_chunks, d_outs, nc,
                                                                            d_ids, d_dict_len, d_err);
        fr.launches++;
        if (n_pairs) {
            k_pq_scan_pages<<<(n_pairs * 32 + 127) / 128, 128, 0, sm>>>(d_pages, d_chunks, d_pairs, n_pairs, d_totals + 8, d_err);
            fr.launches++;
        }
    }

    if (n_pairs == 0) {
        if (np > 0) {
            k_pq_expand<false><<<np, kExpThreads, 0, sm>>>(d_pages, d_dicts, d_chunks, d_outs, nc, d_ids, d_vstart,
                                                           d_dict_off, d_dict_len);
            fr.launches++;
        }
    } else {
        SmallReads rb(sm);
        pg_status rs = rb.add(pair_tot.data(), d_totals + 8, sizeof(int64_t) * n_pairs);
        if (!rs) rs = rb.add(h_tot, d_totals, sizeof(int64_t) * 8);
        if (rs) return rs;
        SideStream *side = nullptr;
        { pg_status st = side_stream(&side); if (st) return st; }
        side_sync.s = side->s;
        PG_CUDA(cudaEventRecord(side->fork, sm));
        const bool main_early = dict_entries == 0;
        if (np > 0) {
            PG_CUDA(cudaStreamWaitEvent(side->s, side->fork, 0));
            k_pq_walk_values<<<(np + kWvWarps * 32 - 1) / (kWvWarps * 32), kWvWarps * 32, 0, side->s>>>(
                d_pages, np, d_chunks, d_vstart, d_err);
            fr.launches++;
            if (main_early) {
                k_pq_expand<false><<<np, kExpThreads, 0, sm>>>(d_pages, d_dicts, d_chunks, d_outs, nc, d_ids, d_vstart,
                                                               d_dict_off, d_dict_len);
                fr.launches++;
            }
        }
        PG_HOST_MARK("enqueue");
        rs = rb.finish(side->fork);
        if (!rs) rs = kernel_error((int)(h_tot[6] & 0xffffffff), "parquet");
        if (rs) return rs;
        PG_HOST_MARK("readback2");
        std::vector<int64_t> payload((size_t)n_runs * nc, 0);
        for (const PqPair &pr : ct.pairs) payload[(size_t)pr.run * nc + pr.col] = pair_tot[pr.idx];
        { pg_status st = b.alloc_payload(payload); if (st) return st; }
        fill_outs();
        if (main_early) {
            pg_status ts = small_h2d(d_outs2, outs.data(), sizeof(PqOut) * outs.size(), side->s);
            if (ts) return ts;
        } else {
            pg_status ts = small_h2d(d_outs2, outs.data(), sizeof(PqOut) * outs.size(), sm);
            if (ts) return ts;
            PG_CUDA(cudaEventRecord(side->tables, sm));
            PG_CUDA(cudaStreamWaitEvent(side->s, side->tables, 0));
            if (np > 0) {
                k_pq_expand<false><<<np, kExpThreads, 0, sm>>>(d_pages, d_dicts, d_chunks, d_outs2, nc, d_ids, d_vstart,
                                                               d_dict_off, d_dict_len);
                fr.launches++;
            }
        }
        if (np > 0) {
            k_pq_expand<true><<<np, kExpThreads, 0, side->s>>>(d_pages, d_dicts, d_chunks, d_outs2, nc, d_ids, d_vstart,
                                                               d_dict_off, d_dict_len);
            fr.launches++;
        }
        PG_CUDA(cudaEventRecord(side->join, side->s));
        PG_CUDA(cudaStreamWaitEvent(sm, side->join, 0));
#ifdef PG_WALK_TIMING
        if (np > 0) walk_timing_dump();
#endif
        PG_HOST_MARK("payload");
    }
    if (any_empty && n_pairs) {
        k_pq_zero_first_offset<<<(n_runs * nc + 127) / 128, 128, 0, sm>>>(d_outs, n_runs * nc);
        fr.launches++;
    }
    meta.clear();
    std::vector<pq::FileMetaData>().swap(own_meta);
    { pg_status st = fr.finish(d_err, out_runs, info); if (st) return st; }
    if (info) {
        info->n_chunks = n_chunks;
        info->n_data_pages = np;
        info->n_dictionary_pages = nd;
    }
    return PG_OK;
}


struct PqReader {
    std::shared_ptr<const Schema> schema;
    pq::FileMetaData meta;
    std::vector<uint8_t> file;
    int64_t n_rows = 0;
    int n_data_pages = 0, n_dict_pages = 0;
    float ms_decode = 0;
    int launches = 0;
};

static Table<PqReader> g_pq(5);

static pg_status pq_open(uint64_t schema, const uint8_t *bytes, int64_t size, uint64_t *out) {
    std::shared_ptr<Schema> s = g_schemas.get(schema);
    if (!s || !bytes || !out) return fail(PG_ERR_INVALID, "bad schema handle or null argument");
    auto rd = std::make_unique<PqReader>();
    rd->schema = s;
    try {
        rd->meta = pq::parse_footer(bytes, size);
    } catch (const std::exception &e) {
        return fail(PG_ERR_FORMAT, e.what());
    }
    Scratch scratch(nullptr);
    RunBuilder b(s, 1, scratch, "parquet");
    pg_status st = map_file_schema(b, rd->meta, 0);
    if (st) return st;
    const pg_file_desc file{bytes, size, PG_MEM_HOST, 0};
    ChunkTables ct;
    st = build_chunk_tables(s.get(), &file, {bytes}, {&rd->meta}, b, ct);
    if (st) return st;
    for (int c = 0; c < (int)ct.chunks.size(); c++) {
        st = kernel_error(pq_walk_chunk<false>(ct.chunks.data(), c, nullptr, nullptr, nullptr), "parquet");
        if (st) return st;
        rd->n_data_pages += ct.chunks[c].n_pages;
        rd->n_dict_pages += ct.chunks[c].n_dicts;
    }
    rd->n_rows = rd->meta.num_rows;
    rd->file.assign(bytes, bytes + size);
    *out = g_pq.put(std::move(rd));
    return PG_OK;
}

static pg_status pq_read_run(PqReader *rd, uint64_t *out_run) {
    const pg_file_desc file{rd->file.data(), (int64_t)rd->file.size(), PG_MEM_HOST, 0};
    pg_section_info info;
    pg_status st = decode_section(rd->schema, &file, 1, 1, nullptr, nullptr, out_run, &info, &rd->meta);
    if (st) return st;
    rd->ms_decode = info.ms_decode;
    rd->launches = info.launches;
    return PG_OK;
}



__global__ void k_dv_keep(const uint8_t *deleted, int64_t n_bits, int64_t n, int32_t *keep) {
    int64_t i = (int64_t)blockIdx.x * blockDim.x + threadIdx.x;
    if (i >= n) return;
    const bool del = i < n_bits && ((deleted[i >> 3] >> (i & 7)) & 1);
    keep[i] = del ? 0 : 1;
}
__global__ void k_dv_sources(const int32_t *incl, int64_t n, int32_t *src) {
    int64_t i = (int64_t)blockIdx.x * blockDim.x + threadIdx.x;
    if (i >= n) return;
    const int32_t cur = incl[i], prev = i ? incl[i - 1] : 0;
    if (cur != prev) src[cur - 1] = (int32_t)i;
}
__global__ void k_dv_gather_fixed(const void *in, int width, const int32_t *src, int64_t m, void *out) {
    int64_t j = (int64_t)blockIdx.x * blockDim.x + threadIdx.x;
    if (j >= m) return;
    store_fixed(out, width, j, load_fixed(in, width, src[j]));
}
__global__ void k_dv_gather_bits(const uint8_t *in, const int32_t *src, int64_t m, uint32_t *out) {
    int64_t j = (int64_t)blockIdx.x * blockDim.x + threadIdx.x;
    const bool v = j < m && valid_bit(in, src[j]);
    const unsigned w = __ballot_sync(0xffffffffu, v);
    if ((threadIdx.x & 31) == 0 && j < m) out[j >> 5] = w;
}
__global__ void k_dv_lengths(const int32_t *offs, const int32_t *src, int64_t m, int32_t *out_offsets) {
    int64_t j = (int64_t)blockIdx.x * blockDim.x + threadIdx.x;
    if (j == 0) out_offsets[0] = 0;
    if (j >= m) return;
    out_offsets[1 + j] = offs[src[j] + 1] - offs[src[j]];
}
__global__ void k_dv_copy_bytes(const uint8_t *data, const int32_t *offs, const int32_t *src, const int32_t *out_offsets,
                                uint8_t *out, int64_t m) {
    int64_t row = ((int64_t)blockIdx.x * blockDim.x + threadIdx.x) >> 3;
    if (row >= m) return;
    const uint8_t *s = data + offs[src[row]];
    const int o0 = out_offsets[row], o1 = out_offsets[row + 1];
    for (int b = o0 + (threadIdx.x & 7); b < o1; b += 8) out[b] = s[b - o0];
}

static pg_status apply_deletion_vector(uint64_t run_h, const uint8_t *deleted, int64_t n_bits, uint64_t *out_run) {
    std::shared_ptr<Run> in = g_runs.get(run_h);
    if (!in || !out_run || (n_bits > 0 && !deleted)) return fail(PG_ERR_INVALID, "unknown run handle or null argument");
    pg_status st = ensure_device();
    if (st) return st;
    const Schema *s = in->schema.get();
    const int nc = s->n_cols();
    const int64_t n = in->n_rows;
    if (n_bits < 0) return fail(PG_ERR_INVALID, "negative deletion vector size");
    cudaStream_t sm = 0;
    Scratch scratch(sm);
    const int64_t nb = std::max<int64_t>((n + 4095) / 4096, 1);
    uint8_t *d_del = (uint8_t *)scratch.take((size_t)(n_bits + 7) / 8 + 16);
    int32_t *d_incl = (int32_t *)scratch.take(sizeof(int32_t) * (size_t)(n + 1));
    int64_t *d_sums = (int64_t *)scratch.take(sizeof(int64_t) * (size_t)nb);
    int32_t *d_err = (int32_t *)scratch.take(16);
    if (!d_del || !d_incl || !d_sums || !d_err) return oom("deletion vector", "the row scan", sizeof(int32_t) * (size_t)n);
    PG_CUDA(cudaMemsetAsync(d_err, 0, 4, sm));
    if (n_bits > 0) PG_CUDA(cudaMemcpyAsync(d_del, deleted, (size_t)(n_bits + 7) / 8, cudaMemcpyHostToDevice, sm));
    int64_t m = 0;
    if (n > 0) {
        k_dv_keep<<<(int)((n + 255) / 256), 256, 0, sm>>>(d_del, n_bits, n, d_incl);
        launch_inclusive_scan(d_incl, n, d_sums, d_err, sm);
        int32_t last = 0;
        PG_CUDA(cudaMemcpyAsync(&last, d_incl + n - 1, 4, cudaMemcpyDeviceToHost, sm));
        PG_CUDA(cudaStreamSynchronize(sm));
        m = last;
    }
    int32_t *d_src = (int32_t *)scratch.take(sizeof(int32_t) * (size_t)std::max<int64_t>(m, 1));
    if (!d_src) return oom("deletion vector", "the row sources", sizeof(int32_t) * (size_t)m);
    if (n > 0) k_dv_sources<<<(int)((n + 255) / 256), 256, 0, sm>>>(d_incl, n, d_src);
    RunBuilder b(in->schema, 1, scratch, "deletion vector");
    b.place_file(0, m);
    std::vector<uint8_t> bitmap(nc), no_zero(nc, 0);
    for (int c = 0; c < nc; c++) {
        b.read[c] = in->cols[c].data || in->cols[c].offsets;
        bitmap[c] = in->cols[c].validity != nullptr;
    }
    st = b.alloc(bitmap, no_zero);
    if (st) return st;
    const int gm = (int)((std::max<int64_t>(m, 1) + 255) / 256);
    for (int c = 0; c < nc; c++) {
        if (!b.read[c]) continue;
        const DevColumn &ic = in->cols[c];
        const OutColumn &oc = b.out[c];
        if (oc.validity && m > 0) k_dv_gather_bits<<<gm, 256, 0, sm>>>(ic.validity, d_src, m, oc.validity);
        if (!is_varlen(s->field(c).type)) {
            if (m > 0) k_dv_gather_fixed<<<gm, 256, 0, sm>>>(ic.data, type_width(s->field(c).type), d_src, m, oc.data);
        } else {
            k_dv_lengths<<<gm, 256, 0, sm>>>(ic.offsets, d_src, m, oc.offsets);
            launch_offsets_scan(oc.offsets, m, d_sums, d_err, sm);
        }
    }
    std::vector<int32_t> totals(nc, 0);
    for (int c = 0; c < nc; c++)
        if (b.out[c].offsets && m > 0)
            PG_CUDA(cudaMemcpyAsync(&totals[c], b.out[c].offsets + m, 4, cudaMemcpyDeviceToHost, sm));
    int32_t herr = 0;
    PG_CUDA(cudaMemcpyAsync(&herr, d_err, 4, cudaMemcpyDeviceToHost, sm));
    PG_CUDA(cudaStreamSynchronize(sm));
    st = b.alloc_payload(std::vector<int64_t>(totals.begin(), totals.end()));
    if (st) return st;
    for (int c = 0; c < nc; c++)
        if (b.out[c].offsets && m > 0)
            k_dv_copy_bytes<<<(int)((m * 8 + 255) / 256), 256, 0, sm>>>((const uint8_t *)in->cols[c].data, in->cols[c].offsets,
                                                                        d_src, b.out[c].offsets, (uint8_t *)b.out[c].data, m);
    PG_CUDA(cudaStreamSynchronize(sm));
    PG_CUDA(cudaGetLastError());
    st = kernel_error(herr, "deletion vector");
    if (st) return st;
    b.finish(out_run, 0, nullptr);
    return PG_OK;
}


}

using namespace pg;

extern "C" {

pg_status pg_parquet_open(uint64_t schema, const uint8_t *file_bytes, int64_t size, uint64_t *out_reader) {
    return pq_open(schema, file_bytes, size, out_reader);
}

pg_status pg_parquet_describe(uint64_t reader, pg_parquet_info *out) {
    std::shared_ptr<PqReader> rd = g_pq.get(reader);
    if (!rd || !out) return fail(PG_ERR_INVALID, "unknown parquet reader handle");
    out->n_rows = rd->n_rows;
    out->n_row_groups = (int32_t)rd->meta.row_groups.size();
    out->n_columns = rd->schema->n_cols();
    out->n_data_pages = rd->n_data_pages;
    out->n_dictionary_pages = rd->n_dict_pages;
    out->ms_decode = rd->ms_decode;
    out->launches = rd->launches;
    return PG_OK;
}

pg_status pg_parquet_read_run(uint64_t reader, uint64_t *out_run) {
    std::shared_ptr<PqReader> rd = g_pq.get(reader);
    if (!rd || !out_run) return fail(PG_ERR_INVALID, "unknown parquet reader handle");
    pg_status st = ensure_device();
    if (st) return st;
    return pq_read_run(rd.get(), out_run);
}

pg_status pg_parquet_read_section(uint64_t schema, const pg_file_desc *files, int32_t n_files, int32_t n_runs,
                                  const char *const *column_names, const uint8_t *read_columns, uint64_t *out_runs,
                                  pg_section_info *info) {
    std::shared_ptr<const Schema> s;
    pg_status st = check_section_args(schema, files, n_files, n_runs, out_runs, &s);
    if (st || n_runs == 0) return st;
    st = ensure_device();
    if (st) return st;
    return decode_section(s, files, n_files, n_runs, column_names, read_columns, out_runs, info);
}

pg_status pg_run_apply_deletion_vector(uint64_t run, const uint8_t *deleted_bitmap, int64_t n_bits, uint64_t *out_run) {
    return apply_deletion_vector(run, deleted_bitmap, n_bits, out_run);
}

pg_status pg_parquet_free(uint64_t reader) {
    return g_pq.take(reader) ? PG_OK : fail(PG_ERR_INVALID, "unknown parquet reader handle");
}

}
```

paimon_b200/csrc/parquet_meta.cc:

```cpp
#include "parquet_meta.h"

#include <algorithm>
#include <stdexcept>

namespace pq {

namespace {

struct Reader {
    const uint8_t *p, *end;
    Reader(const uint8_t *b, int64_t n) : p(b), end(b + n) {}

    uint8_t byte() {
        if (p >= end) throw std::runtime_error("parquet: truncated thrift data");
        return *p++;
    }
    uint64_t varint() {
        if (p < end && !(*p & 0x80)) return *p++;
        uint64_t v = 0;
        int shift = 0;
        while (true) {
            uint8_t b = byte();
            v |= (uint64_t)(b & 0x7f) << shift;
            if (!(b & 0x80)) return v;
            shift += 7;
            if (shift > 63) throw std::runtime_error("parquet: bad varint");
        }
    }
    int64_t zigzag() {
        uint64_t v = varint();
        return (int64_t)(v >> 1) ^ -(int64_t)(v & 1);
    }
    std::string binary() {
        uint64_t n = varint();
        if ((uint64_t)(end - p) < n) throw std::runtime_error("parquet: truncated binary");
        std::string s((const char *)p, (size_t)n);
        p += n;
        return s;
    }
    void skip_binary() {
        uint64_t n = varint();
        if ((uint64_t)(end - p) < n) throw std::runtime_error("parquet: truncated binary");
        p += n;
    }
    bool field(int16_t &last_id, int &type) {
        uint8_t h = byte();
        if (h == CT_STOP) return false;
        int delta = h >> 4;
        type = h & 0x0f;
        if (delta == 0) last_id = (int16_t)zigzag();
        else last_id = (int16_t)(last_id + delta);
        return true;
    }
    void list_header(int &elem_type, uint32_t &size) {
        uint8_t h = byte();
        elem_type = h & 0x0f;
        size = h >> 4;
        if (size == 15) size = (uint32_t)varint();
    }
    void skip(int type) {
        switch (type) {
            case CT_TRUE: case CT_FALSE: return;
            case CT_BYTE: byte(); return;
            case CT_I16: case CT_I32: case CT_I64: varint(); return;
            case CT_DOUBLE: if (end - p < 8) throw std::runtime_error("parquet: truncated double"); p += 8; return;
            case CT_BINARY: skip_binary(); return;
            case CT_LIST: case CT_SET: {
                int et; uint32_t n;
                list_header(et, n);
                for (uint32_t i = 0; i < n; i++) skip_elem(et);
                return;
            }
            case CT_MAP: {
                uint32_t n = (uint32_t)varint();
                if (n == 0) return;
                uint8_t kv = byte();
                for (uint32_t i = 0; i < n; i++) { skip_elem(kv >> 4); skip_elem(kv & 0x0f); }
                return;
            }
            case CT_STRUCT: {
                int16_t id = 0;
                int t;
                while (field(id, t)) skip(t);
                return;
            }
            default: throw std::runtime_error("parquet: unknown thrift type");
        }
    }
    void skip_elem(int type) {
        if (type == CT_TRUE || type == CT_FALSE) { byte(); return; }
        skip(type);
    }
};

SchemaElement read_schema_element(Reader &r) {
    SchemaElement e;
    int16_t id = 0;
    int t;
    while (r.field(id, t)) {
        switch (id) {
            case 1: e.type = (int32_t)r.zigzag(); break;
            case 2: e.type_length = (int32_t)r.zigzag(); break;
            case 3: e.repetition = (int32_t)r.zigzag(); break;
            case 4: e.name = r.binary(); break;
            case 5: e.num_children = (int32_t)r.zigzag(); break;
            case 6: e.converted_type = (int32_t)r.zigzag(); break;
            default: r.skip(t);
        }
    }
    return e;
}

ColumnChunk read_column_meta(Reader &r) {
    ColumnChunk c;
    int16_t id = 0;
    int t;
    while (r.field(id, t)) {
        switch (id) {
            case 1: c.type = (int32_t)r.zigzag(); break;
            case 2: {
                int et; uint32_t n;
                r.list_header(et, n);
                c.encodings.reserve(std::min<uint32_t>(n, 16));
                for (uint32_t i = 0; i < n; i++) c.encodings.push_back((int32_t)r.zigzag());
                break;
            }
            case 3: {
                int et; uint32_t n;
                r.list_header(et, n);
                c.path.reserve(std::min<uint32_t>(n, 16));
                for (uint32_t i = 0; i < n; i++) c.path.push_back(r.binary());
                break;
            }
            case 4: c.codec = (int32_t)r.zigzag(); break;
            case 5: c.num_values = r.zigzag(); break;
            case 6: c.total_uncompressed_size = r.zigzag(); break;
            case 7: c.total_compressed_size = r.zigzag(); break;
            case 9: c.data_page_offset = r.zigzag(); break;
            case 11: c.dictionary_page_offset = r.zigzag(); break;
            default: r.skip(t);
        }
    }
    return c;
}

ColumnChunk read_column_chunk(Reader &r) {
    ColumnChunk c;
    int16_t id = 0;
    int t;
    bool have = false;
    while (r.field(id, t)) {
        if (id == 3 && t == CT_STRUCT) { c = read_column_meta(r); have = true; }
        else r.skip(t);
    }
    if (!have) throw std::runtime_error("parquet: column chunk without meta_data");
    return c;
}

RowGroup read_row_group(Reader &r) {
    RowGroup g;
    int16_t id = 0;
    int t;
    while (r.field(id, t)) {
        switch (id) {
            case 1: {
                int et; uint32_t n;
                r.list_header(et, n);
                g.columns.reserve(std::min<uint32_t>(n, 4096));
                for (uint32_t i = 0; i < n; i++) g.columns.push_back(read_column_chunk(r));
                break;
            }
            case 2: g.total_byte_size = r.zigzag(); break;
            case 3: g.num_rows = r.zigzag(); break;
            default: r.skip(t);
        }
    }
    return g;
}

FileMetaData parse_footer_thrift(const uint8_t *footer, int64_t flen) {
    Reader r(footer, flen);
    FileMetaData m;
    int16_t id = 0;
    int t;
    while (r.field(id, t)) {
        switch (id) {
            case 1: m.version = (int32_t)r.zigzag(); break;
            case 2: {
                int et; uint32_t n;
                r.list_header(et, n);
                m.schema.reserve(std::min<uint32_t>(n, 4096));
                for (uint32_t i = 0; i < n; i++) m.schema.push_back(read_schema_element(r));
                break;
            }
            case 3: m.num_rows = r.zigzag(); break;
            case 4: {
                int et; uint32_t n;
                r.list_header(et, n);
                m.row_groups.reserve(std::min<uint32_t>(n, 4096));
                for (uint32_t i = 0; i < n; i++) m.row_groups.push_back(read_row_group(r));
                break;
            }
            case 6: m.created_by = r.binary(); break;
            default: r.skip(t);
        }
    }
    return m;
}

int64_t footer_length(const uint8_t *tail8) {
    if (tail8[4] != 'P' || tail8[5] != 'A' || tail8[6] != 'R' || tail8[7] != '1')
        throw std::runtime_error("parquet: missing PAR1 magic (encrypted or not a Parquet file)");
    return (int64_t)((uint32_t)tail8[0] | ((uint32_t)tail8[1] << 8) | ((uint32_t)tail8[2] << 16) | ((uint32_t)tail8[3] << 24));
}

}

FileMetaData parse_footer(const uint8_t *file, int64_t size) {
    if (size < 12 || file[0] != 'P' || file[1] != 'A' || file[2] != 'R' || file[3] != '1')
        throw std::runtime_error("parquet: missing PAR1 magic (encrypted or not a Parquet file)");
    const int64_t flen = footer_length(file + size - 8);
    if (flen + 12 > size) throw std::runtime_error("parquet: bad footer length");
    return parse_footer_thrift(file + size - 8 - flen, flen);
}

std::vector<FileMetaData> read_footers(RangeReader &rd, const std::vector<uint64_t> &sizes) {
    const size_t nf = sizes.size();
    std::vector<uint8_t> tails(8 * nf);
    for (size_t f = 0; f < nf; f++) {
        if (sizes[f] < 12) throw std::runtime_error("parquet: missing PAR1 magic (encrypted or not a Parquet file)");
        rd.read((int)f, sizes[f] - 8, 8, &tails[8 * f]);
    }
    rd.flush();
    std::vector<std::vector<uint8_t>> footers(nf);
    for (size_t f = 0; f < nf; f++) {
        const int64_t flen = footer_length(&tails[8 * f]);
        if ((uint64_t)flen + 12 > sizes[f]) throw std::runtime_error("parquet: bad footer length");
        footers[f].resize((size_t)flen);
        rd.read((int)f, sizes[f] - 8 - (uint64_t)flen, (uint64_t)flen, footers[f].data());
    }
    rd.flush();
    std::vector<FooterBytes> spans(nf);
    for (size_t f = 0; f < nf; f++) spans[f] = FooterBytes{footers[f].data(), (int64_t)footers[f].size()};
    return parse_footers(spans);
}

std::vector<FileMetaData> parse_footers(const std::vector<FooterBytes> &footers) {
    std::vector<FileMetaData> m(footers.size());
    for (size_t f = 0; f < footers.size(); f++) m[f] = parse_footer_thrift(footers[f].bytes, footers[f].size);
    return m;
}

}
```

paimon_b200/csrc/parquet_meta.h:

```cpp
#pragma once

#include <stdint.h>

#include <string>
#include <vector>

#include "range_reader.h"

namespace pq {

using pg::RangeReader;

enum PhysType { T_BOOLEAN = 0, T_INT32 = 1, T_INT64 = 2, T_INT96 = 3, T_FLOAT = 4, T_DOUBLE = 5, T_BYTE_ARRAY = 6,
                T_FIXED_LEN_BYTE_ARRAY = 7 };
enum Encoding { E_PLAIN = 0, E_PLAIN_DICTIONARY = 2, E_RLE = 3, E_BIT_PACKED = 4, E_DELTA_BINARY_PACKED = 5,
                E_DELTA_LENGTH_BYTE_ARRAY = 6, E_DELTA_BYTE_ARRAY = 7, E_RLE_DICTIONARY = 8, E_BYTE_STREAM_SPLIT = 9 };
enum Codec { C_UNCOMPRESSED = 0, C_SNAPPY = 1, C_GZIP = 2, C_LZO = 3, C_BROTLI = 4, C_LZ4 = 5, C_ZSTD = 6, C_LZ4_RAW = 7 };
enum PageType { P_DATA = 0, P_INDEX = 1, P_DICTIONARY = 2, P_DATA_V2 = 3 };
enum Repetition { R_REQUIRED = 0, R_OPTIONAL = 1, R_REPEATED = 2 };
enum TType { CT_STOP = 0, CT_TRUE = 1, CT_FALSE = 2, CT_BYTE = 3, CT_I16 = 4, CT_I32 = 5, CT_I64 = 6, CT_DOUBLE = 7,
             CT_BINARY = 8, CT_LIST = 9, CT_SET = 10, CT_MAP = 11, CT_STRUCT = 12 };

struct SchemaElement {
    int32_t type = -1;
    int32_t type_length = 0;
    int32_t repetition = 0;
    std::string name;
    int32_t num_children = 0;
    int32_t converted_type = -1;
};

struct ColumnChunk {
    int32_t type = -1;
    int32_t codec = 0;
    int64_t num_values = 0;
    int64_t total_uncompressed_size = 0;
    int64_t total_compressed_size = 0;
    int64_t data_page_offset = 0;
    int64_t dictionary_page_offset = 0;
    std::vector<int32_t> encodings;
    std::vector<std::string> path;
    int64_t start() const {
        return (dictionary_page_offset > 0 && dictionary_page_offset < data_page_offset) ? dictionary_page_offset
                                                                                        : data_page_offset;
    }
};

struct RowGroup {
    int64_t num_rows = 0;
    int64_t total_byte_size = 0;
    std::vector<ColumnChunk> columns;
};

struct FileMetaData {
    int32_t version = 0;
    int64_t num_rows = 0;
    std::vector<SchemaElement> schema;
    std::vector<RowGroup> row_groups;
    std::string created_by;
};

FileMetaData parse_footer(const uint8_t *file, int64_t size);
std::vector<FileMetaData> read_footers(RangeReader &rd, const std::vector<uint64_t> &sizes);
struct FooterBytes {
    const uint8_t *bytes;
    int64_t size;
};
std::vector<FileMetaData> parse_footers(const std::vector<FooterBytes> &footers);

inline void put_varint(std::vector<uint8_t> &b, uint64_t v) {
    while (v >= 0x80) { b.push_back((uint8_t)(v | 0x80)); v >>= 7; }
    b.push_back((uint8_t)v);
}

struct ThriftWriter {
    std::vector<uint8_t> b;
    std::vector<int> last{0};
    void varint(uint64_t v) { put_varint(b, v); }
    void zigzag(int64_t v) { varint(((uint64_t)v << 1) ^ (uint64_t)(v >> 63)); }
    void field(int id, int type) {
        int d = id - last.back();
        if (d > 0 && d <= 15) b.push_back((uint8_t)((d << 4) | type));
        else { b.push_back((uint8_t)type); zigzag(id); }
        last.back() = id;
    }
    void i32(int id, int32_t v) { field(id, CT_I32); zigzag(v); }
    void i64(int id, int64_t v) { field(id, CT_I64); zigzag(v); }
    void binary(const void *p, size_t n) { varint(n); b.insert(b.end(), (const uint8_t *)p, (const uint8_t *)p + n); }
    void bin(int id, const void *p, size_t n) { field(id, CT_BINARY); binary(p, n); }
    void str(int id, const std::string &s) { bin(id, s.data(), s.size()); }
    void list(int id, int elem_type, size_t n) {
        field(id, CT_LIST);
        if (n < 15) b.push_back((uint8_t)((n << 4) | elem_type));
        else { b.push_back((uint8_t)(0xF0 | elem_type)); varint(n); }
    }
    void struct_field(int id) { field(id, CT_STRUCT); last.push_back(0); }
    void struct_elem() { last.push_back(0); }
    void end() { b.push_back(CT_STOP); last.pop_back(); }
};

}
```

paimon_b200/csrc/pg_internal.h:

```cpp
#pragma once

#include <cuda_runtime.h>
#include <stdint.h>
#include <stdio.h>

#include <chrono>
#include <memory>
#include <mutex>
#include <string>
#include <unordered_map>
#include <utility>
#include <vector>

#include "device_layout.h"
#include "paimon_gpu.h"
#include "range_reader.h"

namespace pg {

constexpr int kPlanTile = 2048;
constexpr int kTileMax = 2 * kPlanTile;
constexpr int kSampleStride = 16;
constexpr int kThreads = 256;
constexpr int kMaxCols = 256;

constexpr uint16_t kPlanSlotMask = 0x0FFF;
constexpr int kPlanOpShift = 12;
constexpr uint16_t kPlanEmit = 0x4000;
constexpr uint16_t kPlanHead = 0x8000;
enum : int { OP_NOOP = 0, OP_UPD = 1, OP_SET = 2, OP_RETRACT = 3 };

enum : int {
    KERR_NONE = 0,
    KERR_TILE_OVERFLOW = 1,
    KERR_PU_DELETE = 2,
    KERR_FIRST_ROW_RETRACT = 3,
    KERR_AGG_RETRACT = 4,
    KERR_OFFSET_OVERFLOW = 5,
    KERR_DIV_ZERO = 6,
    KERR_BAD_PAGE = 7,
    KERR_PQ_HEADER = 8,
    KERR_PQ_ENCODING = 9,
    KERR_PQ_NO_DICT = 10,
    KERR_PQ_ROWS = 11,
    KERR_PQ_DICT_ID = 12,
    KERR_PQ_LEVELS = 13,
    KERR_DEC_DIV_ZERO = 14,
    KERR_DEC_DIV_UNDEFINED = 15,
    KERR_DEC_NON_TERMINATING = 16
};

struct Schema {
    int n_key = 0, n_val = 0;
    std::vector<pg_field> key_fields, val_fields;
    int n_cols() const { return n_key + 2 + n_val; }
    pg_field field(int c) const {
        if (c < n_key) return key_fields[c];
        if (c == n_key) return pg_field{PG_INT64, 0};
        if (c == n_key + 1) return pg_field{PG_INT8, 0};
        return val_fields[c - n_key - 2];
    }
};

struct Spec {
    std::shared_ptr<const Schema> schema;
    int engine = 0, ignore_delete = 0, remove_record_on_delete = 0, drop_delete = 0;
    std::vector<int32_t> seq_fields;
    int seq_ascending = 1;
    std::vector<int32_t> agg;
    std::vector<uint8_t> ignore_retract;
    std::vector<int32_t> group_seq_start, group_seq_fields, field_group;
    std::vector<uint8_t> group_partial_delete;
    std::vector<uint8_t> read_fields;
    std::vector<int32_t> decimal;
    int n_groups() const { return group_seq_start.empty() ? 0 : (int)group_seq_start.size() - 1; }
};

struct DevColumn {
    const void *data = nullptr;
    const int32_t *offsets = nullptr;
    const uint8_t *validity = nullptr;
};

void *buf_take(size_t bytes, size_t *got);
void buf_give(void *p, size_t bytes);

class DeviceBuffer {
 public:
    DeviceBuffer() = default;
    explicit DeviceBuffer(size_t bytes) { p_ = buf_take(bytes, &n_); }
    DeviceBuffer(DeviceBuffer &&o) noexcept : p_(o.p_), n_(o.n_) { o.p_ = nullptr; o.n_ = 0; }
    DeviceBuffer &operator=(DeviceBuffer &&o) noexcept {
        std::swap(p_, o.p_);
        std::swap(n_, o.n_);
        return *this;
    }
    DeviceBuffer(const DeviceBuffer &) = delete;
    DeviceBuffer &operator=(const DeviceBuffer &) = delete;
    ~DeviceBuffer() { if (p_) buf_give(p_, n_); }
    unsigned char *get() const { return (unsigned char *)p_; }
    explicit operator bool() const { return p_ != nullptr; }

 private:
    void *p_ = nullptr;
    size_t n_ = 0;
};

inline size_t align256(size_t x) { return (x + 255) & ~(size_t)255; }

struct Run {
    Run(std::shared_ptr<const Schema> s, int64_t rows)
        : schema(std::move(s)), n_rows(rows), cols(schema->n_cols()), varlen_bytes(schema->n_cols(), 0),
          varlen_base(schema->n_cols(), 0) {}
    Run(const Run &) = delete;
    Run &operator=(const Run &) = delete;
    std::shared_ptr<const Schema> schema;
    int64_t n_rows;
    std::vector<DevColumn> cols;
    std::vector<int64_t> varlen_bytes;
    std::vector<int64_t> varlen_base;
    std::vector<DeviceBuffer> bufs;
    std::shared_ptr<const Run> source;
    int64_t bytes_h2d = 0;
};

struct Scratch {
    explicit Scratch(cudaStream_t s) : stream(s) {}
    ~Scratch() { if (!bufs.empty() || !runs.empty()) cudaStreamSynchronize(stream); }
    void *take(size_t bytes) {
        DeviceBuffer b(bytes ? bytes : 256);
        if (!b) return nullptr;
        bufs.push_back(std::move(b));
        return bufs.back().get();
    }
    cudaStream_t stream;
    std::vector<DeviceBuffer> bufs;
    std::vector<std::unique_ptr<Run>> runs;
};

pg_status oom(const char *who, const char *what, size_t bytes);

struct OutColumn {
    void *data = nullptr;
    int32_t *offsets = nullptr;
    uint32_t *validity = nullptr;
};

pg_status check_file_desc(const pg_file_desc &f);
pg_status check_section_args(uint64_t schema, const pg_file_desc *files, int n_files, int n_runs, const uint64_t *out_runs,
                             std::shared_ptr<const Schema> *s);
pg_status file_image(Scratch &scratch, const uint8_t *bytes, int64_t size, const char *who, const uint8_t **out);

struct RunBuilder {
    RunBuilder(std::shared_ptr<const Schema> s, int n_runs, Scratch &scratch, const char *who)
        : schema(std::move(s)), nc(schema->n_cols()), scratch(scratch), who(who), read(nc, 1), run_rows(n_runs, 0),
          missing((size_t)n_runs * nc, 0), with_rows((size_t)n_runs * nc, 0) {}
    pg_status read_columns(const uint8_t *read_cols, const char *const *names);
    pg_status add_file(int run, int64_t rows, const std::vector<std::string> &cols);
    int64_t place_file(int run, int64_t rows) {
        const int64_t row0 = run_rows[run];
        run_rows[run] += rows;
        return row0;
    }
    pg_status check_runs() const;
    pg_status alloc(const std::vector<uint8_t> &bitmap, const std::vector<uint8_t> &zero);
    pg_status alloc_payload(const std::vector<int64_t> &payload);
    void finish(uint64_t *out_runs, int64_t bytes_h2d, pg_section_info *info);

    const std::shared_ptr<const Schema> schema;
    const int nc;
    Scratch &scratch;
    const char *who;
    std::vector<uint8_t> read;
    const char *const *names = nullptr;
    std::vector<int64_t> run_rows;
    std::vector<std::vector<int>> file_col;
    std::vector<int64_t> file_row0;
    std::vector<uint8_t> missing;
    std::vector<uint8_t> with_rows;
    std::vector<OutColumn> out;
    int64_t decoded_bytes = 0;
};

#ifdef PG_HOST_TIMING
struct HostMarks {
    explicit HostMarks(const char *who) : who(who), t0(std::chrono::steady_clock::now()), last(t0) {}
    void mark(const char *phase) {
        const auto t = std::chrono::steady_clock::now();
        line += std::string(" ") + phase + " " + std::to_string(std::chrono::duration<double, std::milli>(t - last).count());
        last = t;
    }
    ~HostMarks() {
        mark("rest");
        fprintf(stderr, "[host timing] %s:%s total %.4f\n", who, line.c_str(),
                std::chrono::duration<double, std::milli>(last - t0).count());
    }
    const char *who;
    std::chrono::steady_clock::time_point t0, last;
    std::string line;
};
#define PG_HOST_MARKS(who) pg::HostMarks pg_host_marks_(who)
#define PG_HOST_MARK(phase) pg_host_marks_.mark(phase)
#else
#define PG_HOST_MARKS(who) do {} while (0)
#define PG_HOST_MARK(phase) do {} while (0)
#endif

struct SectionTimer {
    cudaEvent_t e0 = nullptr, e1 = nullptr;
    ~SectionTimer() {
        if (e0) cudaEventDestroy(e0);
        if (e1) cudaEventDestroy(e1);
    }
    float ms() const {
        float ms = 0;
        cudaEventElapsedTime(&ms, e0, e1);
        return ms;
    }
};

struct SectionFrame {
    SectionFrame(std::shared_ptr<const Schema> s, int n_runs, const char *who);
    pg_status start(const uint8_t *read_cols, const char *const *names);
    pg_status place(const pg_file_desc *files, int n_files);
    pg_status finish(const int32_t *d_err, uint64_t *out_runs, pg_section_info *info);

    const cudaStream_t stream;
    Scratch scratch;
    RunBuilder b;
    SectionTimer tm;
    int launches = 0;
    std::vector<const uint8_t *> d_file;
    int64_t file_bytes = 0, h2d = 0, page_bytes = 0;
};

template <typename T>
class Table {
 public:
    explicit Table(uint64_t tag) : tag_(tag << 56) {}
    uint64_t put(std::shared_ptr<T> p) {
        std::lock_guard<std::mutex> g(mu_);
        const uint64_t h = tag_ | next_++;
        map_[h] = std::move(p);
        return h;
    }
    std::shared_ptr<T> get(uint64_t h) {
        std::lock_guard<std::mutex> g(mu_);
        auto it = map_.find(h);
        return it == map_.end() ? nullptr : it->second;
    }
    std::shared_ptr<T> take(uint64_t h) {
        std::lock_guard<std::mutex> g(mu_);
        auto node = map_.extract(h);
        return node.empty() ? nullptr : std::move(node.mapped());
    }

 private:
    std::mutex mu_;
    std::unordered_map<uint64_t, std::shared_ptr<T>> map_;
    uint64_t next_ = 1;
    const uint64_t tag_;
};
extern Table<Schema> g_schemas;
extern Table<Run> g_runs;

pg_status ensure_device();
cudaStream_t copy_stream();
struct Merge;
struct BatchColumns {
    std::shared_ptr<const Schema> schema;
    std::vector<DevColumn> cols;
    int64_t n_rows = 0;
    std::shared_ptr<const Run> run;
    std::shared_ptr<Merge> merge;
};
pg_status batch_columns(uint64_t handle, BatchColumns *out);


struct ColDesc {
    int32_t type;
    int32_t width;
    int16_t nullable;
    int16_t retract;
    int32_t mode;
    int32_t agg;
    int32_t varlen_index;
    int32_t group;
    int32_t decimal;
};
static_assert(sizeof(ColDesc) == 32, "ColDesc is staged in shared memory by the emit kernel");
enum : int { CM_SELECT = 0, CM_FOLD = 1, CM_KEY = 2, CM_SEQ = 3, CM_KIND = 4, CM_GVAL = 5, CM_GSEQ = 6, CM_GAGG = 7 };
enum : int { RT_OK = 0, RT_IGNORE = 1, RT_ERROR = 2 };

struct MergeFlags {
    int32_t engine, ignore_delete, remove_record_on_delete, drop_delete;
};

struct KeyDesc {
    int32_t n_fields;
    int32_t exact;
    int32_t type[PG_MAX_KEY_FIELDS];
    int32_t width[PG_MAX_KEY_FIELDS];
};

struct KeySrc {
    const void *const *data;
    const int32_t *const *offsets;
};

inline int type_width(int t) {
    switch (t) {
        case PG_INT8: case PG_BOOL: return 1;
        case PG_INT16: return 2;
        case PG_INT32: case PG_FLOAT: return 4;
        case PG_INT64: case PG_DOUBLE: return 8;
        default: return 0;
    }
}
static bool type_ok(int t) { return t >= PG_INT8 && t <= PG_BINARY; }
inline bool is_varlen(int t) { return t == PG_STRING || t == PG_BINARY; }

void set_error(const std::string &msg);
pg_status fail(pg_status code, const std::string &msg);
pg_status kernel_error(int code, const char *who);

#define PG_CUDA(expr)                                                                      \
    do {                                                                                   \
        cudaError_t _e = (expr);                                                           \
        if (_e != cudaSuccess)                                                             \
            return pg::fail(PG_ERR_CUDA, std::string(#expr) + ": " + cudaGetErrorString(_e)); \
    } while (0)


struct LevelView {
    int64_t count[PG_MAX_RUNS];
    int64_t row0[PG_MAX_RUNS];
    int64_t stride;
};

struct MergeLaunch {
    int k;
    KeyDesc key;
    KeySrc ks;
    cudaStream_t stream;
    int32_t *err;
    const int *skip;
};

void launch_partition(const MergeLaunch &ml, const LevelView &lv, const uint64_t *splitter_keys,
                      const uint64_t *splitter_refs, int q, int n_tiles, int64_t *bounds);
void launch_key_lcp(const MergeLaunch &ml, const LevelView &lv0, int *skip);
void launch_merge_keys(const MergeLaunch &ml, const LevelView &lv, const int64_t *bounds, int n_tiles,
// ... 112 lines not shown
```

Measured before the change: 887.5 million.

## Parse Parquet footers on device and build chunk table with a GPU kernel

Adds a device-side Thrift footer parser that runs one block per file: the footer is staged into shared memory and parsed into a compact record log plus a chunk array. A warp-per-column kernel then builds the chunk table and walks the pages on the GPU. Only a small header is copied back to the host, replacing full host parsing of FileMetaData. This is meant to cut host-side footer parsing and host-to-device transfer of chunk metadata when there are many footers. The host path is kept as a fallback when one footer dominates the total size, at the cost of extra kernel launches and small synchronous readbacks.

```diff
diff --git a/paimon_b200/csrc/api.cu b/paimon_b200/csrc/api.cu
--- a/paimon_b200/csrc/api.cu
+++ b/paimon_b200/csrc/api.cu
@@ -660,6 +660,9 @@
         {KERR_PQ_NO_DICT, PG_ERR_FORMAT, "dictionary-encoded page without dictionary"},
         {KERR_PQ_ROWS, PG_ERR_FORMAT, "page row counts do not add up"},
         {KERR_PQ_DICT_ID, PG_ERR_FORMAT, "dictionary id outside the dictionary"},
+        {KERR_PQ_FOOTER, PG_ERR_FORMAT,
+         "a footer's column chunk does not match its row group, its file or the schema (value count, page offset or "
+         "physical type)"},
         {KERR_PQ_ENCODING, PG_ERR_UNSUPPORTED,
          "a page uses a value encoding the device decoder does not implement (PLAIN, dictionary, DELTA_BINARY_PACKED "
          "integers and RLE booleans are decoded)"},
diff --git a/paimon_b200/csrc/parquet_decode.cu b/paimon_b200/csrc/parquet_decode.cu
--- a/paimon_b200/csrc/parquet_decode.cu
+++ b/paimon_b200/csrc/parquet_decode.cu
@@ -5,6 +5,7 @@
 
 #include "device_utils.cuh"
 #include "parquet_meta.h"
+#include "parquet_footer.cuh"
 #include "inflate_device.cuh"
 #include "lz4_device.cuh"
 #include "snappy_device.cuh"
@@ -77,70 +78,6 @@
     return v;
 }
 
-
-struct TRd {
-    const uint8_t *p, *end;
-    int bad;
-    __host__ __device__ uint32_t byte() {
-        if (p >= end) { bad = 1; return 0; }
-        return *p++;
-    }
-    __host__ __device__ uint64_t varint() {
-        uint64_t v = 0;
-        for (int sh = 0; sh < 70; sh += 7) {
-            const uint32_t b = byte();
-            v |= (uint64_t)(b & 0x7f) << sh;
-            if (!(b & 0x80)) return v;
-        }
-        bad = 1;
-        return v;
-    }
-    __host__ __device__ int64_t zz() {
-        const uint64_t v = varint();
-        return (int64_t)(v >> 1) ^ -(int64_t)(v & 1);
-    }
-    __host__ __device__ int field(int &id) {
-        const uint32_t h = byte();
-        if (h == 0 || bad) return 0;
-        const int d = (int)(h >> 4);
-        if (d == 0) id = (int)zz(); else id += d;
-        return (int)(h & 15);
-    }
-    __host__ __device__ void advance(uint64_t n) {
-        if ((uint64_t)(end - p) < n) { bad = 1; p = end; } else p += n;
-    }
-    __host__ __device__ void skip_flat(int t, bool in_container) {
-        switch (t) {
-            case 1: case 2: if (in_container) byte(); return;
-            case 3: byte(); return;
-            case 4: case 5: case 6: varint(); return;
-            case 7: advance(8); return;
-            case 8: advance(varint()); return;
-            case 9: case 10: {
-                const uint32_t h = byte();
-                const int et = (int)(h & 15);
-                uint64_t n = h >> 4;
-                if (n == 15) n = varint();
-                if (et == 9 || et == 10 || et == 11 || et == 12) { if (n) bad = 1; return; }
-                for (uint64_t i = 0; i < n && !bad; i++) skip_flat(et, true);
-                return;
-            }
-            case 11: { if (varint() != 0) bad = 1; return; }
-            default: bad = 1; return;
-        }
-    }
-    __host__ __device__ void skip(int t) {
-        if (t != 12) { skip_flat(t, false); return; }
-        int depth = 1;
-        while (depth > 0 && !bad) {
-            const uint32_t h = byte();
-            if (h == 0) { depth--; continue; }
-            if ((h >> 4) == 0) zz();
-            const int ft = (int)(h & 15);
-            if (ft == 12) depth++; else skip_flat(ft, false);
-        }
-    }
-};
 
 struct PqHeader {
     int type, unc, comp, nv, enc, def_enc, def_len, rep_len, is_compressed, hdr;
@@ -1155,6 +1092,82 @@
     if (i < n && outs[i].offsets) outs[i].offsets[0] = 0;
 }
 
+struct PqFooterJob {
+    const uint8_t *footer;
+    int64_t len;
+    PfOut out;
+};
+constexpr int kFooterThreads = 256;
+constexpr int kFooterStage = 64 * 1024;
+constexpr int64_t kFooterHead = 4096;
+
+__global__ void __launch_bounds__(kFooterThreads) k_pq_footers(const PqFooterJob *jobs, int stage) {
+    extern __shared__ __align__(16) uint8_t s_footer[];
+    const PqFooterJob j = jobs[blockIdx.x];
+    const uint8_t *src = j.footer;
+    if (j.len + 16 <= stage) {
+        const uint8_t *a0 = (const uint8_t *)((uintptr_t)j.footer & ~(uintptr_t)15);
+        const int skew = (int)((uintptr_t)j.footer & 15);
+        const int n = skew + (int)j.len;
+        for (int o = threadIdx.x * 16; o < n; o += kFooterThreads * 16) {
+            if (o >= skew && o + 16 <= n) *(uint4 *)(s_footer + o) = *(const uint4 *)(a0 + o);
+            else for (int b = max(o, skew); b < min(o + 16, n); b++) s_footer[b] = a0[b];
+        }
+        __syncthreads();
+        src = s_footer + skew;
+    }
+    if (threadIdx.x == 0) pq_parse_footer(src, j.len, j.out);
+}
+
+__host__ __device__ inline int phys_width_of(int phys) {
+    return phys == pq::T_INT32 || phys == pq::T_FLOAT ? 4 : (phys == pq::T_INT64 || phys == pq::T_DOUBLE ? 8 : 0);
+}
+
+struct PqChunkSrc {
+    const uint8_t *file;
+    int64_t file_size;
+    int64_t row0;
+    const PfChunk *chunks;
+    int32_t n_cols, fc;
+    int32_t group0, n_groups;
+    int32_t out0;
+    int32_t col, run, file_idx;
+    int32_t max_def, phys, cast, pad;
+};
+struct PqGroupRow {
+    int64_t rows, row0;
+    int32_t out, pad;
+};
+
+__global__ void k_pq_chunk_table(const PqChunkSrc *src, int n_src, const PqGroupRow *groups, PqChunk *chunks, int32_t *err) {
+    const int e = (int)(((int64_t)blockIdx.x * blockDim.x + threadIdx.x) >> 5), lane = threadIdx.x & 31;
+    if (e >= n_src) return;
+    const PqChunkSrc s = src[e];
+    for (int g = lane; g < s.n_groups; g += 32) {
+        const PqGroupRow gr = groups[s.group0 + g];
+        const PfChunk cc = s.chunks[(int64_t)g * s.n_cols + s.fc];
+        bool ok = cc.num_values == gr.rows;
+        if (gr.rows == 0) {
+            if (!ok) pq_err(err, KERR_PQ_FOOTER);
+            continue;
+        }
+        ok = ok && cc.start >= 4 && cc.start < s.file_size && cc.type == s.phys;
+        PqChunk ch;
+        memset(&ch, 0, sizeof(ch));
+        ch.base = s.file + (ok ? cc.start : 0);
+        ch.avail = ok ? pq_min64(cc.total_compressed_size > 0 ? cc.total_compressed_size : s.file_size, s.file_size - cc.start) : 0;
+        ch.num_values = ok ? cc.num_values : 0;
+        ch.row0 = s.row0 + gr.row0;
+        ch.col = s.col; ch.run = s.run; ch.file = s.file_idx; ch.codec = cc.codec;
+        ch.max_def = s.max_def; ch.phys = s.phys; ch.phys_width = phys_width_of(s.phys); ch.cast = s.cast;
+        const int c = s.out0 + gr.out;
+        chunks[c] = ch;
+        if (!ok) { pq_err(err, KERR_PQ_FOOTER); continue; }
+        const int code = pq_walk_chunk<false>(chunks, c, nullptr, nullptr, nullptr);
+        if (code != KERR_NONE) pq_err(err, code);
+    }
+}
+
 
 static int phys_cast(int pg_t, int phys) {
     switch (pg_t) {
@@ -1167,11 +1180,39 @@
         default: return -1;
     }
 }
-static int phys_width_of(int phys) {
-    return phys == pq::T_INT32 || phys == pq::T_FLOAT ? 4 : (phys == pq::T_INT64 || phys == pq::T_DOUBLE ? 8 : 0);
-}
-
-static pg_status map_file_schema(RunBuilder &b, const pq::FileMetaData &m, int run) {
+
+struct FooterView {
+    struct Elem {
+        int32_t type, repetition, num_children;
+        std::string name;
+    };
+    struct Group {
+        int64_t rows;
+        int32_t cols;
+    };
+    int64_t num_rows = 0;
+    std::vector<Elem> schema;
+    std::vector<Group> groups;
+    int32_t bad_codec = -1;
+    int64_t bad_codec_at = -1;
+};
+
+static FooterView footer_view(const pq::FileMetaData &m) {
+    FooterView v;
+    v.num_rows = m.num_rows;
+    for (const pq::SchemaElement &e : m.schema) v.schema.push_back({e.type, e.repetition, e.num_children, e.name});
+    int64_t k = 0;
+    for (const pq::RowGroup &g : m.row_groups) {
+        v.groups.push_back({g.num_rows, (int32_t)g.columns.size()});
+        for (const pq::ColumnChunk &cc : g.columns) {
+            if (v.bad_codec < 0 && !pf_codec_on_device(cc.codec)) { v.bad_codec = cc.codec; v.bad_codec_at = k; }
+            k++;
+        }
+    }
+    return v;
+}
+
+static pg_status map_file_schema(RunBuilder &b, const FooterView &m, int run) {
     if (m.schema.empty()) return fail(PG_ERR_FORMAT, "parquet: empty schema");
     const int nleaf = (int)m.schema.size() - 1;
     if (m.schema[0].num_children != nleaf)
@@ -1186,19 +1227,19 @@
     for (int c = 0; c < b.nc; c++) {
         const int fc = b.file_col.back()[c];
         if (fc < 0) continue;
-        const pq::SchemaElement &e = m.schema[fc + 1];
+        const FooterView::Elem &e = m.schema[fc + 1];
         if (phys_cast(b.schema->field(c).type, e.type) < 0)
             return fail(PG_ERR_UNSUPPORTED, "parquet: column " + e.name + " has a physical type the device decoder "
                                             "does not map to the table type");
     }
-    for (const pq::RowGroup &g : m.row_groups) {
-        if ((int)g.columns.size() != nleaf) return fail(PG_ERR_FORMAT, "parquet: row group with a different column count");
-        for (const pq::ColumnChunk &cc : g.columns)
-            if (cc.codec != pq::C_UNCOMPRESSED && cc.codec != pq::C_SNAPPY && cc.codec != pq::C_ZSTD && cc.codec != pq::C_GZIP &&
-                cc.codec != pq::C_LZ4)
-                return fail(PG_ERR_UNSUPPORTED, "parquet: compression codec " + std::to_string(cc.codec) +
-                                                " is not decoded on device (UNCOMPRESSED, SNAPPY, ZSTD, GZIP and Hadoop-framed LZ4 = 5 are); write with "
-                                                "'file.compression'='zstd' / 'snappy' / 'gzip' / 'lz4' / 'none' or let the Java side decompress");
+    int64_t chunk0 = 0;
+    for (const FooterView::Group &g : m.groups) {
+        if (g.cols != nleaf) return fail(PG_ERR_FORMAT, "parquet: row group with a different column count");
+        if (m.bad_codec_at >= chunk0 && m.bad_codec_at < chunk0 + g.cols)
+            return fail(PG_ERR_UNSUPPORTED, "parquet: compression codec " + std::to_string(m.bad_codec) +
+                                            " is not decoded on device (UNCOMPRESSED, SNAPPY, ZSTD, GZIP and Hadoop-framed LZ4 = 5 are); write with "
+                                            "'file.compression'='zstd' / 'snappy' / 'gzip' / 'lz4' / 'none' or let the Java side decompress");
+        chunk0 += g.cols;
     }
     return PG_OK;
 }
@@ -1327,9 +1368,199 @@
     ~SideSync() { if (s) cudaStreamSynchronize(s); }
 };
 
+struct SectionFooters {
+    std::vector<FooterView> views;
+    std::vector<const PfChunk *> chunks;
+    bool any_snappy = false, any_lz4 = false, any_zstd = false, any_delta = false;
+    bool on_device = false;
+};
+constexpr int64_t kFooterFanout = 8;
+
+static const char *footer_error(int status) {
+    switch (status) {
+        case PF_ERR_NO_META: return "parquet: column chunk without meta_data";
+        case PF_ERR_DEPTH: return "parquet: footer with containers nested more than 32 deep";
+        case PF_ERR_CAPACITY: return "parquet: footer with more elements than its length can hold";
+        default: return "parquet: malformed or truncated footer";
+    }
+}
+
+static pg_status section_footers(SectionFrame &fr, const pg_file_desc *files, int nf, SectionFooters &out) {
+    cudaStream_t sm = fr.stream;
+    static const char *const kNoMagic = "parquet: missing PAR1 magic (encrypted or not a Parquet file)";
+    std::vector<uint8_t> tails(8 * (size_t)nf);
+    {
+        SmallReads rb(sm);
+        bool any_device = false;
+        for (int f = 0; f < nf; f++) {
+            const pg_file_desc &fd = files[f];
+            if (fd.size < 12) return fail(PG_ERR_FORMAT, kNoMagic);
+            if (fd.mem == PG_MEM_HOST) {
+                if (memcmp(fd.bytes, "PAR1", 4) != 0) return fail(PG_ERR_FORMAT, kNoMagic);
+                memcpy(&tails[8 * (size_t)f], fd.bytes + fd.size - 8, 8);
+            } else {
+                pg_status rs = rb.add(&tails[8 * (size_t)f], fd.bytes + fd.size - 8, 8);
+                if (rs) return rs;
+                any_device = true;
+            }
+        }
+        if (any_device) { pg_status rs = rb.finish(); if (rs) return rs; }
+    }
+    std::vector<int64_t> flen(nf);
+    int64_t longest = 0, all = 0;
+    for (int f = 0; f < nf; f++) {
+        try {
+            flen[f] = pq::footer_length(&tails[8 * (size_t)f]);
+        } catch (const std::exception &e) {
+            return fail(PG_ERR_FORMAT, e.what());
+        }
+        if (flen[f] + 12 > files[f].size) return fail(PG_ERR_FORMAT, "parquet: bad footer length");
+        longest = std::max(longest, flen[f]);
+        all += flen[f];
+    }
+    const bool on_device = longest * kFooterFanout <= all;
+    out.on_device = on_device;
+
+    std::vector<PqFooterJob> jobs(nf);
+    PqFooterJob *d_jobs = nullptr;
+    uint8_t *d_head = nullptr;
+    auto carve = [&](void *base) {
+        Carver cv(base);
+        if (on_device) {
+            d_jobs = cv.take<PqFooterJob>((size_t)nf);
+            d_head = cv.take<uint8_t>((size_t)nf * kFooterHead);
+        }
+        for (int f = 0; f < nf; f++) {
+            PfOut &o = jobs[f].out;
+            o.head = on_device && base ? d_head + (size_t)f * kFooterHead : nullptr;
+            o.head_cap = kFooterHead;
+            o.log_cap = pf_log_cap(flen[f]);
+            o.over = on_device ? cv.take<uint8_t>((size_t)std::max<int64_t>(o.log_cap - kFooterHead, 0)) : nullptr;
+            o.chunk_cap = pf_chunk_cap(flen[f]);
+            o.chunks = cv.take<PfChunk>((size_t)o.chunk_cap);
+            jobs[f].footer = fr.d_file[f] + files[f].size - 8 - flen[f];
+            jobs[f].len = flen[f];
+        }
+        return cv.bytes();
+    };
+    const size_t ws_bytes = carve(nullptr);
+    void *ws = fr.scratch.take(ws_bytes);
+    if (!ws) return oom("parquet", "the footer records", ws_bytes);
+    carve(ws);
+
+    std::vector<PfFile> hdr(nf);
+    std::vector<std::vector<uint8_t>> logs(nf);
+    if (on_device) {
+        { pg_status ts = small_h2d(d_jobs, jobs.data(), sizeof(PqFooterJob) * nf, sm); if (ts) return ts; }
+        int stage = 0;
+        for (int f = 0; f < nf; f++)
+            if (flen[f] + 16 <= kFooterStage) stage = std::max(stage, (int)((flen[f] + 16 + 15) & ~(int64_t)15));
+        if (stage > 48 * 1024)
+            PG_CUDA(cudaFuncSetAttribute(k_pq_footers, cudaFuncAttributeMaxDynamicSharedMemorySize, kFooterStage));
+        k_pq_footers<<<nf, kFooterThreads, stage, sm>>>(d_jobs, stage);
+        fr.launches++;
+        std::vector<uint8_t> head((size_t)nf * kFooterHead);
+        {
+            SmallReads rb(sm);
+            pg_status rs = rb.add(head.data(), d_head, head.size());
+            if (!rs) rs = rb.finish();
+            if (rs) return rs;
+        }
+        SmallReads rb(sm);
+        bool more = false;
+        for (int f = 0; f < nf; f++) {
+            memcpy(&hdr[f], &head[(size_t)f * kFooterHead], sizeof(PfFile));
+            const PfFile &h = hdr[f];
+            if (h.status != PF_OK) return fail(PG_ERR_FORMAT, footer_error(h.status));
+            if (h.log_bytes < (int64_t)sizeof(PfFile) || h.log_bytes > jobs[f].out.log_cap)
+                return fail(PG_ERR_INTERNAL, "parquet: a footer's record log is out of its bounds");
+            const uint8_t *h0 = &head[(size_t)f * kFooterHead];
+            logs[f].assign(h0, h0 + std::min(h.log_bytes, kFooterHead));
+            if (h.log_bytes > kFooterHead) {
+                logs[f].resize((size_t)h.log_bytes);
+                pg_status rs = rb.add(logs[f].data() + kFooterHead, jobs[f].out.over, (size_t)(h.log_bytes - kFooterHead));
+                if (rs) return rs;
+                more = true;
+            }
+        }
+        if (more) { pg_status rs = rb.finish(); if (rs) return rs; }
+    } else {
+        std::vector<std::vector<uint8_t>> footers(nf);
+        {
+            SmallReads rb(sm);
+            bool any_device = false;
+            for (int f = 0; f < nf; f++) {
+                if (files[f].mem == PG_MEM_HOST) continue;
+                footers[f].resize((size_t)flen[f]);
+                pg_status rs = rb.add(footers[f].data(), jobs[f].footer, (size_t)flen[f]);
+                if (rs) return rs;
+                any_device = true;
+            }
+            if (any_device) { pg_status rs = rb.finish(); if (rs) return rs; }
+        }
+        for (int f = 0; f < nf; f++) {
+            const uint8_t *src = files[f].mem == PG_MEM_HOST ? files[f].bytes + files[f].size - 8 - flen[f] : footers[f].data();
+            logs[f].resize((size_t)jobs[f].out.log_cap);
+            std::vector<PfChunk> chunks((size_t)jobs[f].out.chunk_cap);
+            const PfOut o{logs[f].data(), logs[f].data(), jobs[f].out.log_cap, jobs[f].out.log_cap, chunks.data(),
+                          jobs[f].out.chunk_cap};
+            const int st = pq_parse_footer(src, flen[f], o);
+            if (st != PF_OK) return fail(PG_ERR_FORMAT, footer_error(st));
+            memcpy(&hdr[f], logs[f].data(), sizeof(PfFile));
+            logs[f].resize((size_t)hdr[f].log_bytes);
+            if (hdr[f].n_chunks) {
+                pg_status ts = small_h2d(jobs[f].out.chunks, chunks.data(), sizeof(PfChunk) * hdr[f].n_chunks, sm);
+                if (ts) return ts;
+            }
+        }
+    }
+    out.views.assign(nf, FooterView());
+    out.chunks.assign(nf, nullptr);
+    for (int f = 0; f < nf; f++) {
+        const PfFile &h = hdr[f];
+        const std::vector<uint8_t> &lg = logs[f];
+        FooterView &v = out.views[f];
+        v.num_rows = h.num_rows;
+        v.bad_codec = h.bad_codec;
+        v.bad_codec_at = h.bad_codec_at;
+        size_t pos = sizeof(PfFile);
+        auto i32 = [&] { int32_t x; memcpy(&x, &lg[pos], 4); pos += 4; return x; };
+        bool ok = true;
+        while (ok && pos < lg.size()) {
+            if (lg.size() - pos < 4) { ok = false; break; }
+            const int32_t tag = i32();
+            if (tag == PF_TAG_SCHEMA && lg.size() - pos >= kPfSchemaRec - 4) {
+                FooterView::Elem e;
+                e.type = i32(); e.repetition = i32(); e.num_children = i32();
+                const uint32_t nl = (uint32_t)i32();
+                if (lg.size() - pos < nl) { ok = false; break; }
+                e.name.assign((const char *)&lg[pos], nl);
+                pos += nl;
+                v.schema.push_back(std::move(e));
+            } else if (tag == PF_TAG_GROUP && lg.size() - pos >= kPfGroupRec - 4) {
+                const int32_t cols = i32();
+                int64_t rows;
+                memcpy(&rows, &lg[pos], 8);
+                pos += 8;
+                v.groups.push_back({rows, cols});
+            } else {
+                ok = false;
+            }
+        }
+        if (!ok || (int64_t)v.schema.size() != h.n_schema || (int64_t)v.groups.size() != h.n_groups)
+            return fail(PG_ERR_INTERNAL, "parquet: a footer's record log does not parse");
+        out.chunks[f] = jobs[f].out.chunks;
+        out.any_snappy |= (h.codecs >> pq::C_SNAPPY) & 1;
+        out.any_lz4 |= (h.codecs >> pq::C_LZ4) & 1;
+        out.any_zstd |= ((h.codecs >> pq::C_ZSTD) | (h.codecs >> pq::C_GZIP)) & 1;
+        out.any_delta |= h.any_delta != 0;
+    }
+    return PG_OK;
+}
+
 static pg_status decode_section(const std::shared_ptr<const Schema> &s, const pg_file_desc *files, int nf, int n_runs,
                                 const char *const *names, const uint8_t *read_cols, uint64_t *out_runs,
-                                pg_section_info *info, const pq::FileMetaData *footer0 = nullptr) {
+                                pg_section_info *info) {
     const int nc = s->n_cols();
     SectionFrame fr(s, n_runs, "parquet");
     SideSync side_sync;
@@ -1339,37 +1570,69 @@
     { pg_status st = fr.start(read_cols, names); if (st) return st; }
 
     { pg_status st = fr.place(files, nf); if (st) return st; }
-    std::vector<pq::FileMetaData> own_meta(nf);
-    std::vector<const pq::FileMetaData *> meta(nf, nullptr);
-    if (footer0) meta[0] = footer0;
-    DeviceRanges rd(sm, files, nf);
-    try {
-        if (!rd.files.empty()) {
-            std::vector<pq::FileMetaData> m = pq::read_footers(rd, rd.sizes);
-            for (size_t i = 0; i < rd.files.size(); i++) own_meta[rd.files[i]] = std::move(m[i]);
-        }
-        for (int f = 0; f < nf; f++) {
-            if (meta[f]) continue;
-            if (files[f].mem == PG_MEM_HOST) own_meta[f] = pq::parse_footer(files[f].bytes, files[f].size);
-            meta[f] = &own_meta[f];
-        }
-    } catch (const std::exception &e) {
-        return rd.st ? rd.st : fail(PG_ERR_FORMAT, e.what());
-    }
-    PG_HOST_MARK("footers");
+    SectionFooters ft;
+    { pg_status st = section_footers(fr, files, nf, ft); if (st) return st; }
+    PG_HOST_MARK(ft.on_device ? "footers(device)" : "footers(host)");
     std::vector<uint8_t> any_optional(nc, 0);
     for (int f = 0; f < nf; f++) {
-        pg_status st = map_file_schema(b, *meta[f], files[f].run);
+        pg_status st = map_file_schema(b, ft.views[f], files[f].run);
         if (st) return st;
         for (int c = 0; c < nc; c++) {
             const int fc = b.file_col[f][c];
-            if (fc == -1 || (fc >= 0 && meta[f]->schema[fc + 1].repetition == pq::R_OPTIONAL)) any_optional[c] = 1;
+            if (fc == -1 || (fc >= 0 && ft.views[f].schema[fc + 1].repetition == pq::R_OPTIONAL)) any_optional[c] = 1;
         }
     }
     { pg_status st = b.check_runs(); if (st) return st; }
-    ChunkTables ct;
-    { pg_status st = build_chunk_tables(s.get(), files, fr.d_file, meta, b, ct); if (st) return st; }
-    const int n_chunks = (int)ct.chunks.size(), n_pairs = (int)ct.pairs.size();
+
+    std::vector<PqGroupRow> groups;
+    std::vector<int32_t> group0(nf), out_groups(nf);
+    for (int f = 0; f < nf; f++) {
+        group0[f] = (int32_t)groups.size();
+        int64_t row0 = 0;
+        int32_t out = 0;
+        for (const FooterView::Group &g : ft.views[f].groups) {
+            groups.push_back(PqGroupRow{g.rows, row0, g.rows != 0 ? out++ : -1, 0});
+            row0 += g.rows;
+        }
+        out_groups[f] = out;
+        if (row0 != ft.views[f].num_rows) return fail(PG_ERR_FORMAT, "parquet: row group row counts do not add up");
+    }
+    std::vector<std::vector<int>> run_files(n_runs);
+    for (int f = 0; f < nf; f++) run_files[files[f].run].push_back(f);
+    std::vector<PqChunkSrc> srcs;
+    std::vector<PqPair> pairs;
+    int64_t n_chunks64 = 0, pair_rows = 0;
+    for (int r = 0; r < n_runs; r++) {
+        for (int c = 0; c < nc; c++) {
+            if (!b.read[c]) continue;
+            const int chunk0 = (int)n_chunks64;
+            for (int f : run_files[r]) {
+                const int fc = b.file_col[f][c];
+                if (fc < 0) continue;
+                const FooterView &v = ft.views[f];
+                const FooterView::Elem &e = v.schema[fc + 1];
+                PqChunkSrc src;
+                memset(&src, 0, sizeof(src));
+                src.file = fr.d_file[f]; src.file_size = files[f].size; src.row0 = b.file_row0[f];
+                src.chunks = ft.chunks[f];
+                src.n_cols = (int32_t)v.schema.size() - 1; src.fc = fc;
+                src.group0 = group0[f]; src.n_groups = (int32_t)v.groups.size();
+                src.out0 = (int32_t)n_chunks64;
+                src.col = c; src.run = r; src.file_idx = f;
+                src.max_def = e.repetition == pq::R_OPTIONAL ? 1 : 0;
+                src.phys = e.type;
+                src.cast = phys_cast(s->field(c).type, e.type);
+                srcs.push_back(src);
+                n_chunks64 += out_groups[f];
+            }
+            if (is_varlen(s->field(c).type)) {
+                pairs.push_back(PqPair{r, c, chunk0, (int)n_chunks64, pair_rows, (int)pairs.size(), 0});
+                pair_rows += b.run_rows[r];
+            }
+        }
+        if (n_chunks64 > 0x7fffffffLL) return fail(PG_ERR_UNSUPPORTED, "parquet: too many column chunks in one section");
+    }
+    const int n_chunks = (int)n_chunks64, n_pairs = (int)pairs.size(), n_srcs = (int)srcs.size();
     PG_HOST_MARK("chunk_tables");
 
     { pg_status st = b.alloc(any_optional, b.missing); if (st) return st; }
@@ -1384,12 +1647,16 @@
     const bool any_empty = std::find(b.run_rows.begin(), b.run_rows.end(), 0) != b.run_rows.end();
 
     PqChunk *d_chunks;
+    PqChunkSrc *d_srcs;
+    PqGroupRow *d_groups;
     PqOut *d_outs, *d_outs2;
     PqPair *d_pairs;
     int64_t *d_totals;
     auto carve_tables = [&](void *base) {
         Carver cv(base);
         d_chunks = cv.take<PqChunk>((size_t)std::max(n_chunks, 1));
+        d_srcs = cv.take<PqChunkSrc>((size_t)std::max(n_srcs, 1));
+        d_groups = cv.take<PqGroupRow>(std::max<size_t>(groups.size(), 1));
         d_outs = cv.take<PqOut>(outs.size());
         d_outs2 = cv.take<PqOut>(outs.size());
         d_pairs = cv.take<PqPair>((size_t)std::max(n_pairs, 1));
@@ -1402,15 +1669,22 @@
     carve_tables(tb);
     int32_t *d_err = (int32_t *)(d_totals + 6);
     PG_CUDA(cudaMemsetAsync(d_totals, 0, sizeof(int64_t) * (8 + (size_t)n_pairs), sm));
-    if (n_chunks) { pg_status ts = small_h2d(d_chunks, ct.chunks.data(), sizeof(PqChunk) * n_chunks, sm); if (ts) return ts; }
+    if (n_srcs) {
+        pg_status ts = small_h2d(d_srcs, srcs.data(), sizeof(PqChunkSrc) * n_srcs, sm);
+        if (!ts) ts = small_h2d(d_groups, groups.data(), sizeof(PqGroupRow) * groups.size(), sm);
+        if (ts) return ts;
+    }
     { pg_status ts = small_h2d(d_outs, outs.data(), sizeof(PqOut) * outs.size(), sm); if (ts) return ts; }
-    if (n_pairs) { pg_status ts = small_h2d(d_pairs, ct.pairs.data(), sizeof(PqPair) * n_pairs, sm); if (ts) return ts; }
+    if (n_pairs) { pg_status ts = small_h2d(d_pairs, pairs.data(), sizeof(PqPair) * n_pairs, sm); if (ts) return ts; }
     int64_t h_tot[8] = {0, 0, 0, 0, 0, 0, 0, 0};
     PG_HOST_MARK("tables");
+    if (n_srcs) {
+        k_pq_chunk_table<<<(n_srcs * 32 + 127) / 128, 128, 0, sm>>>(d_srcs, n_srcs, d_groups, d_chunks, d_err);
+        fr.launches++;
+    }
     if (n_chunks) {
-        k_pq_walk<false><<<(n_chunks + 63) / 64, 64, 0, sm>>>(d_chunks, n_chunks, nullptr, nullptr, nullptr, d_err);
         k_pq_chunk_scan<<<1, kScanThreads, 0, sm>>>(d_chunks, n_chunks, d_totals);
-        fr.launches += 2;
+        fr.launches++;
         {
             SmallReads rb(sm);
             pg_status rs = rb.add(h_tot, d_totals, sizeof(int64_t) * 8);
@@ -1426,7 +1700,7 @@
     if (n_pages > 0x7fffffffLL) return fail(PG_ERR_UNSUPPORTED, "parquet: too many pages in one section");
 
     int zs_ctas = 0;
-    if (ct.any_zstd) {
+    if (ft.any_zstd) {
         int dev = 0, sms = 132;
         cudaGetDevice(&dev);
         cudaDeviceGetAttribute(&sms, cudaDevAttrMultiProcessorCount, dev);
@@ -1443,7 +1717,7 @@
         d_dict_off = cv.take<int32_t>((size_t)dict_entries + 1);
         d_dict_len = cv.take<int32_t>((size_t)dict_entries + 1);
         d_ids = cv.take<int32_t>((size_t)ids_entries + 1);
-        d_vstart = cv.take<int32_t>((size_t)(ct.pair_rows + n_pages + n_pairs + 2));
+        d_vstart = cv.take<int32_t>((size_t)(pair_rows + n_pages + n_pairs + 2));
         d_zs_lit = cv.take<uint8_t>((size_t)zs_ctas * kZsWarps * (size_t)(zs::kMaxBlock + 64));
         return cv.bytes();
     };
@@ -1456,16 +1730,16 @@
     if (np > 0) {
         k_pq_walk<true><<<(n_chunks + 63) / 64, 64, 0, sm>>>(d_chunks, n_chunks, d_pages, d_dicts, d_sc, d_err);
         fr.launches++;
-        if (ct.any_snappy || ct.any_lz4) {
+        if (ft.any_snappy || ft.any_lz4) {
             const int64_t th = (int64_t)(np + nd) * 32;
             k_pq_snappy_lz4<<<(unsigned)((th + 127) / 128), 128, 0, sm>>>(d_pages, np, d_dicts, nd, d_chunks, d_err);
             fr.launches++;
         }
-        if (ct.any_zstd && zs_ctas > 0) {
+        if (ft.any_zstd && zs_ctas > 0) {
             k_pq_zstd<<<zs_ctas, kZsWarps * 32, 0, sm>>>(d_pages, np, d_dicts, nd, d_chunks, d_zs_lit, (int32_t *)(d_totals + 7), d_err);
             fr.launches++;
         }
-        if (ct.any_delta) {
+        if (ft.any_delta) {
             k_pq_delta<<<(unsigned)(((int64_t)np * 32 + 127) / 128), 128, 0, sm>>>(d_pages, np, d_chunks, d_err);
             fr.launches++;
         }
@@ -1516,7 +1790,7 @@
         if (rs) return rs;
         PG_HOST_MARK("readback2");
         std::vector<int64_t> payload((size_t)n_runs * nc, 0);
-        for (const PqPair &pr : ct.pairs) payload[(size_t)pr.run * nc + pr.col] = pair_tot[pr.idx];
+        for (const PqPair &pr : pairs) payload[(size_t)pr.run * nc + pr.col] = pair_tot[pr.idx];
         { pg_status st = b.alloc_payload(payload); if (st) return st; }
         fill_outs();
         if (main_early) {
@@ -1549,8 +1823,6 @@
         k_pq_zero_first_offset<<<(n_runs * nc + 127) / 128, 128, 0, sm>>>(d_outs, n_runs * nc);
         fr.launches++;
     }
-    meta.clear();
-    std::vector<pq::FileMetaData>().swap(own_meta);
     { pg_status st = fr.finish(d_err, out_runs, info); if (st) return st; }
     if (info) {
         info->n_chunks = n_chunks;
@@ -1585,7 +1857,7 @@
     }
     Scratch scratch(nullptr);
     RunBuilder b(s, 1, scratch, "parquet");
-    pg_status st = map_file_schema(b, rd->meta, 0);
+    pg_status st = map_file_schema(b, footer_view(rd->meta), 0);
     if (st) return st;
     const pg_file_desc file{bytes, size, PG_MEM_HOST, 0};
     ChunkTables ct;
@@ -1606,7 +1878,7 @@
 static pg_status pq_read_run(PqReader *rd, uint64_t *out_run) {
     const pg_file_desc file{rd->file.data(), (int64_t)rd->file.size(), PG_MEM_HOST, 0};
     pg_section_info info;
-    pg_status st = decode_section(rd->schema, &file, 1, 1, nullptr, nullptr, out_run, &info, &rd->meta);
+    pg_status st = decode_section(rd->schema, &file, 1, 1, nullptr, nullptr, out_run, &info);
     if (st) return st;
     rd->ms_decode = info.ms_decode;
     rd->launches = info.launches;
diff --git a/paimon_b200/csrc/parquet_footer.cuh b/paimon_b200/csrc/parquet_footer.cuh
--- /dev/null
+++ b/paimon_b200/csrc/parquet_footer.cuh
@@ -0,0 +1,348 @@
+#pragma once
+
+#include <stdint.h>
+
+#if defined(__CUDACC__)
+#define PF_HD __host__ __device__
+#else
+#define PF_HD
+#endif
+
+namespace pg {
+
+struct TRd {
+    const uint8_t *p, *end;
+    int bad;
+    PF_HD uint32_t byte() {
+        if (p >= end) { bad = 1; return 0; }
+        return *p++;
+    }
+    PF_HD uint64_t varint() {
+        uint64_t v = 0;
+        for (int sh = 0; sh < 70; sh += 7) {
+            const uint32_t b = byte();
+            v |= (uint64_t)(b & 0x7f) << sh;
+            if (!(b & 0x80)) return v;
+        }
+        bad = 1;
+        return v;
+    }
+    PF_HD int64_t zz() {
+        const uint64_t v = varint();
+        return (int64_t)(v >> 1) ^ -(int64_t)(v & 1);
+    }
+    PF_HD int field(int &id) {
+        const uint32_t h = byte();
+        if (h == 0 || bad) return 0;
+        const int d = (int)(h >> 4);
+        if (d == 0) id = (int)zz(); else id += d;
+        return (int)(h & 15);
+    }
+    PF_HD void advance(uint64_t n) {
+        if ((uint64_t)(end - p) < n) { bad = 1; p = end; } else p += n;
+    }
+    PF_HD void skip_flat(int t, bool in_container) {
+        switch (t) {
+            case 1: case 2: if (in_container) byte(); return;
+            case 3: byte(); return;
+            case 4: case 5: case 6: varint(); return;
+            case 7: advance(8); return;
+            case 8: advance(varint()); return;
+            case 9: case 10: {
+                const uint32_t h = byte();
+                const int et = (int)(h & 15);
+                uint64_t n = h >> 4;
+                if (n == 15) n = varint();
+                if (et == 9 || et == 10 || et == 11 || et == 12) { if (n) bad = 1; return; }
+                for (uint64_t i = 0; i < n && !bad; i++) skip_flat(et, true);
+                return;
+            }
+            case 11: { if (varint() != 0) bad = 1; return; }
+            default: bad = 1; return;
+        }
+    }
+    PF_HD void skip(int t) {
+        if (t != 12) { skip_flat(t, false); return; }
+        int depth = 1;
+        while (depth > 0 && !bad) {
+            const uint32_t h = byte();
+            if (h == 0) { depth--; continue; }
+            if ((h >> 4) == 0) zz();
+            const int ft = (int)(h & 15);
+            if (ft == 12) depth++; else skip_flat(ft, false);
+        }
+    }
+};
+
+
+enum : int32_t {
+    PF_OK = 0,
+    PF_ERR_THRIFT = 1,
+    PF_ERR_NO_META = 2,
+    PF_ERR_DEPTH = 3,
+    PF_ERR_CAPACITY = 4
+};
+constexpr int kPfDepth = 32;
+
+struct PfFile {
+    int32_t status;
+    int32_t n_schema, n_groups, n_chunks;
+    int64_t num_rows;
+    int64_t log_bytes;
+    int32_t bad_codec;
+    int32_t bad_codec_at;
+    uint32_t codecs;
+    int32_t any_delta;
+};
+enum : int32_t { PF_TAG_SCHEMA = 1, PF_TAG_GROUP = 2 };
+constexpr int kPfSchemaRec = 20, kPfGroupRec = 16;
+
+struct PfChunk {
+    int64_t num_values;
+    int64_t start;
+    int64_t total_compressed_size;
+    int32_t type, codec;
+};
+
+struct PfOut {
+    uint8_t *head, *over;
+    int64_t head_cap, log_cap;
+    PfChunk *chunks;
+    int64_t chunk_cap;
+};
+PF_HD inline int64_t pf_log_cap(int64_t flen) { return (int64_t)sizeof(PfFile) + (int64_t)kPfSchemaRec * flen; }
+PF_HD inline int64_t pf_chunk_cap(int64_t flen) { return flen / 3 + 1; }
+
+PF_HD inline bool pf_codec_on_device(int32_t c) { return c == 0 || c == 1 || c == 2 || c == 5 || c == 6; }
+
+struct PfParse {
+    TRd r;
+    const PfOut &o;
+    PfFile f;
+    int64_t log = (int64_t)sizeof(PfFile);
+    int status = PF_OK;
+
+    PF_HD PfParse(const uint8_t *p, int64_t n, const PfOut &out) : r{p, p + n, 0}, o(out) {
+        f.status = PF_OK; f.n_schema = 0; f.n_groups = 0; f.n_chunks = 0; f.num_rows = 0; f.log_bytes = 0;
+        f.bad_codec = -1; f.bad_codec_at = -1; f.codecs = 0; f.any_delta = 0;
+    }
+    PF_HD void fail(int st) {
+        if (status == PF_OK) status = st;
+        r.bad = 1;
+    }
+    PF_HD void put_at(int64_t at, const uint8_t *src, int64_t n) {
+        for (int64_t i = 0; i < n; i++, at++) {
+            if (at < o.head_cap) o.head[at] = src[i]; else o.over[at - o.head_cap] = src[i];
+        }
+    }
+    PF_HD bool room(int64_t n) {
+        if (log + n > o.log_cap) { fail(PF_ERR_CAPACITY); return false; }
+        return true;
+    }
+    PF_HD void put_i32(int32_t v) {
+        const uint8_t b[4] = {(uint8_t)v, (uint8_t)(v >> 8), (uint8_t)(v >> 16), (uint8_t)(v >> 24)};
+        put_at(log, b, 4);
+        log += 4;
+    }
+    PF_HD void put_i64(int64_t v) { put_i32((int32_t)v); put_i32((int32_t)(v >> 32)); }
+
+    PF_HD bool field(int16_t &id, int &t) {
+        const uint32_t h = r.byte();
+        if (h == 0 || r.bad) return false;
+        const int d = (int)(h >> 4);
+        t = (int)(h & 15);
+        id = d == 0 ? (int16_t)r.zz() : (int16_t)(id + d);
+        return !r.bad;
+    }
+    PF_HD uint32_t list_header() {
+        const uint32_t h = r.byte();
+        uint32_t n = h >> 4;
+        if (n == 15) n = (uint32_t)r.varint();
+        return r.bad ? 0 : n;
+    }
+
+    PF_HD void skip(int t) {
+        struct Frame { uint32_t left; uint8_t kind, t0, t1, half; };
+        Frame st[kPfDepth];
+        int sp = 0;
+        bool elem = false;
+        while (!r.bad) {
+            switch (t) {
+                case 1: case 2: if (elem) r.byte(); break;
+                case 3: r.byte(); break;
+                case 4: case 5: case 6: r.varint(); break;
+                case 7: r.advance(8); break;
+                case 8: r.advance(r.varint()); break;
+                case 9: case 10: case 11: case 12: {
+                    if (sp == kPfDepth) { fail(PF_ERR_DEPTH); return; }
+                    Frame &fr = st[sp++];
+                    fr.kind = (uint8_t)t; fr.half = 0; fr.t0 = 0; fr.t1 = 0; fr.left = 0;
+                    if (t == 12) break;
+                    if (t == 11) {
+                        fr.left = (uint32_t)r.varint();
+                        if (fr.left) { const uint32_t kv = r.byte(); fr.t0 = (uint8_t)(kv >> 4); fr.t1 = (uint8_t)(kv & 15); }
+                    } else {
+                        const uint32_t h = r.byte();
+                        fr.t0 = (uint8_t)(h & 15);
+                        fr.left = h >> 4;
+                        if (fr.left == 15) fr.left = (uint32_t)r.varint();
+                    }
+                    break;
+                }
+                default: fail(PF_ERR_THRIFT); return;
+            }
+            bool next = false;
+            while (sp > 0 && !r.bad && !next) {
+                Frame &fr = st[sp - 1];
+                if (fr.kind == 12) {
+                    int16_t id = 0;
+                    int ft = 0;
+                    if (field(id, ft)) { t = ft; elem = false; next = true; } else sp--;
+                } else if (fr.left == 0) {
+                    sp--;
+                } else if (fr.kind == 11) {
+                    t = fr.half ? fr.t1 : fr.t0;
+                    if (fr.half) fr.left--;
+                    fr.half ^= 1;
+                    elem = true;
+                    next = true;
+                } else {
+                    fr.left--;
+                    t = fr.t0;
+                    elem = true;
+                    next = true;
+                }
+            }
+            if (!next) return;
+        }
+    }
+
+    PF_HD void schema_element() {
+        int32_t type = -1, rep = 0, nch = 0;
+        const uint8_t *name = nullptr;
+        uint64_t name_len = 0;
+        int16_t id = 0;
+        int t;
+        while (field(id, t)) {
+            switch (id) {
+                case 1: type = (int32_t)r.zz(); break;
+                case 3: rep = (int32_t)r.zz(); break;
+                case 4: name_len = r.varint(); name = r.p; r.advance(name_len); break;
+                case 5: nch = (int32_t)r.zz(); break;
+                case 2: case 6: r.zz(); break;
+                default: skip(t);
+            }
+        }
+        if (r.bad || !room(kPfSchemaRec + (int64_t)name_len)) return;
+        put_i32(PF_TAG_SCHEMA); put_i32(type); put_i32(rep); put_i32(nch); put_i32((int32_t)name_len);
+        put_at(log, name, (int64_t)name_len);
+        log += (int64_t)name_len;
+        f.n_schema++;
+    }
+
+    PF_HD void column_meta(PfChunk &c, bool &delta) {
+        c.type = -1; c.codec = 0; c.num_values = 0; c.total_compressed_size = 0;
+        int64_t dpo = 0, dico = 0;
+        delta = false;
+        int16_t id = 0;
+        int t;
+        while (field(id, t)) {
+            switch (id) {
+                case 1: c.type = (int32_t)r.zz(); break;
+                case 2: {
+                    const uint32_t n = list_header();
+                    for (uint32_t i = 0; i < n && !r.bad; i++) if ((int32_t)r.zz() == 5) delta = true;
+                    break;
+                }
+                case 3: {
+                    const uint32_t n = list_header();
+                    for (uint32_t i = 0; i < n && !r.bad; i++) r.advance(r.varint());
+                    break;
+                }
+                case 4: c.codec = (int32_t)r.zz(); break;
+                case 5: c.num_values = r.zz(); break;
+                case 6: r.zz(); break;
+                case 7: c.total_compressed_size = r.zz(); break;
+                case 9: dpo = r.zz(); break;
+                case 11: dico = r.zz(); break;
+                default: skip(t);
+            }
+        }
+        c.start = (dico > 0 && dico < dpo) ? dico : dpo;
+    }
+
+    PF_HD void column_chunk() {
+        PfChunk c;
+        bool have = false, delta = false;
+        int16_t id = 0;
+        int t;
+        while (field(id, t)) {
+            if (id == 3 && t == 12) { column_meta(c, delta); have = true; }
+            else skip(t);
+        }
+        if (r.bad) return;
+        if (!have) { fail(PF_ERR_NO_META); return; }
+        if (f.n_chunks >= o.chunk_cap) { fail(PF_ERR_CAPACITY); return; }
+        if (f.bad_codec < 0 && !pf_codec_on_device(c.codec)) { f.bad_codec = c.codec; f.bad_codec_at = f.n_chunks; }
+        if (c.codec >= 0 && c.codec < 32) f.codecs |= 1u << c.codec;
+        if (delta) f.any_delta = 1;
+        o.chunks[f.n_chunks++] = c;
+    }
+
+    PF_HD void row_group() {
+        int64_t rows = 0;
+        int32_t cols = 0;
+        int16_t id = 0;
+        int t;
+        while (field(id, t)) {
+            switch (id) {
+                case 1: {
+                    const uint32_t n = list_header();
+                    for (uint32_t i = 0; i < n && !r.bad; i++) { column_chunk(); cols++; }
+                    break;
+                }
+                case 2: r.zz(); break;
+                case 3: rows = r.zz(); break;
+                default: skip(t);
+            }
+        }
+        if (r.bad || !room(kPfGroupRec)) return;
+        put_i32(PF_TAG_GROUP); put_i32(cols); put_i64(rows);
+        f.n_groups++;
+    }
+
+    PF_HD int run() {
+        int16_t id = 0;
+        int t;
+        while (field(id, t)) {
+            switch (id) {
+                case 1: r.zz(); break;
+                case 2: {
+                    const uint32_t n = list_header();
+                    for (uint32_t i = 0; i < n && !r.bad; i++) schema_element();
+                    break;
+                }
+                case 3: f.num_rows = r.zz(); break;
+                case 4: {
+                    const uint32_t n = list_header();
+                    for (uint32_t i = 0; i < n && !r.bad; i++) row_group();
+                    break;
+                }
+                case 6: r.advance(r.varint()); break;
+                default: skip(t);
+            }
+        }
+        if (r.bad && status == PF_OK) status = PF_ERR_THRIFT;
+        f.status = status;
+        f.log_bytes = log;
+        put_at(0, (const uint8_t *)&f, (int64_t)sizeof(PfFile));
+        return status;
+    }
+};
+
+PF_HD inline int pq_parse_footer(const uint8_t *footer, int64_t n, const PfOut &o) {
+    PfParse ps(footer, n, o);
+    return ps.run();
+}
+
+}
diff --git a/paimon_b200/csrc/parquet_meta.cc b/paimon_b200/csrc/parquet_meta.cc
--- a/paimon_b200/csrc/parquet_meta.cc
+++ b/paimon_b200/csrc/parquet_meta.cc
@@ -208,12 +208,12 @@
     return m;
 }
 
+}
+
 int64_t footer_length(const uint8_t *tail8) {
     if (tail8[4] != 'P' || tail8[5] != 'A' || tail8[6] != 'R' || tail8[7] != '1')
         throw std::runtime_error("parquet: missing PAR1 magic (encrypted or not a Parquet file)");
     return (int64_t)((uint32_t)tail8[0] | ((uint32_t)tail8[1] << 8) | ((uint32_t)tail8[2] << 16) | ((uint32_t)tail8[3] << 24));
-}
-
 }
 
 FileMetaData parse_footer(const uint8_t *file, int64_t size) {
diff --git a/paimon_b200/csrc/parquet_meta.h b/paimon_b200/csrc/parquet_meta.h
--- a/paimon_b200/csrc/parquet_meta.h
+++ b/paimon_b200/csrc/parquet_meta.h
@@ -60,6 +60,7 @@
     std::string created_by;
 };
 
+int64_t footer_length(const uint8_t *tail8);
 FileMetaData parse_footer(const uint8_t *file, int64_t size);
 std::vector<FileMetaData> read_footers(RangeReader &rd, const std::vector<uint64_t> &sizes);
 struct FooterBytes {
diff --git a/paimon_b200/csrc/pg_internal.h b/paimon_b200/csrc/pg_internal.h
--- a/paimon_b200/csrc/pg_internal.h
+++ b/paimon_b200/csrc/pg_internal.h
@@ -47,7 +47,8 @@
     KERR_PQ_LEVELS = 13,
     KERR_DEC_DIV_ZERO = 14,
     KERR_DEC_DIV_UNDEFINED = 15,
-    KERR_DEC_NON_TERMINATING = 16
+    KERR_DEC_NON_TERMINATING = 16,
+    KERR_PQ_FOOTER = 17
 };
 
 struct Schema {
```

Result: faster. 908.7 million (median of 6 runs) (+2.4%).
